# pyamg/pyamg

Hardware: AMD Instinct MI355X
Metric: vcycle_iterations_per_sec (higher is better)
Workload: dtype f64; 1 GPU; 3D 7-pt Poisson 256^3 (16.7M dof) SA V-cycle, symmetric Gauss-Seidel, fp64; key=c3, n=16777216, nnz=117047296, levels=5, cycle=V(1,1), graph=True, parallelism=1 GPU, gs_order=fast, full=False

## Files before the change

### pyamg_amd/csrc/pamg_common.h

```cpp
#pragma once
#include "pamg_host_threads.h"
#include <hip/hip_runtime.h>

#include <cstdint>
#include <cstdio>
#include <cstdlib>
#include <ctime>
#include <algorithm>
#include <atomic>
#include <cstring>
#include <thread>
#include <vector>

#include "../../include/pyamg_amd.h"

#define PAMG_STR2(x) #x
#define PAMG_STR(x) PAMG_STR2(x)
#define PAMG_HIP(expr)                                   \
    do {                                                 \
        hipError_t e__ = (expr);                         \
        if (e__ != hipSuccess) return (int)e__;          \
    } while (0)
#define PAMG_TRY(expr)                                   \
    do {                                                 \
// ... 149 lines not shown
    int use_rowg = 0;
    unsigned char *d_pid = nullptr;
    void *d_ptab = nullptr;
    int npat = 0, pat_lmax = 0;
    unsigned char *d_pmask = nullptr;
    int rm_nu = 0, rm_off[8] = {0, 0, 0, 0, 0, 0, 0, 0};
    unsigned long long rm_val[8] = {0, 0, 0, 0, 0, 0, 0, 0};
    long long rm_walked = 0;
    int rowmask_kz = 8;
    int rowmask_flags = 3;
    int use_rowpat = 1;
    int cap_from_val8 = 0;
    int stream_flags = 0;
    int lds_pad = 0;
    int gran_xcd = 0;
    int gran_cap = 0;
    int gs_mode = 0;
    int tile_G = 0;
    int tile_W = 0;
    int tile_cap = 0;
    int tile_D = 0, tile_Q = -1;
    int tile_part = 1;
    bool tile_default = false;
    int max_row_len = 0;
    int borrowed = 0;
    int gs_prof = 0;
    int gs_order = 0;
    int lane_L = 0, lane_G = 0;
    int lane_flags = 1;
    int line_scan = 1;
    int lane_merge = 0;
    int lanem_rpw = 0;
    int lanem_cluster = 0;
    int lanem_ahead10 = 40;
    int lane_wide = 0;
    int gs_cap = 0;
    int nblk = 0;
    int *d_part[2] = {nullptr, nullptr};
    int npart[2] = {0, 0};
    int64_t part_cols = -1;
    int64_t part_row0[2] = {-1, -1}, part_row1[2] = {-1, -1};
    int4 *d_blkmeta = nullptr;
    double *d_partial = nullptr;
    pamg::GsSchedule *gs[4] = {nullptr, nullptr, nullptr, nullptr};
    pamg_matrix_s *point_twin = nullptr;
    size_t point_twin_bytes = 0;
    bool point_twin_unfit = false;
    pamg::LineSchedule *ls[4] = {nullptr, nullptr, nullptr, nullptr};
    int sym_fused = 1;
    void *d_sym_hf[2] = {nullptr, nullptr}, *d_sym_hb = nullptr;
    unsigned *d_sym_sync = nullptr;
    int sym_cap = 0;
    const void *sym_cap_kernel = nullptr;
    int sym_form = 0, sym_grid = 0;
    long long sym_launches = 0, sym_zero_launches = 0;
    size_t bytes = 0;
};

struct pamg_schwarz_s;
struct pamg_solver_s;
struct pamg_csr_s;

namespace pamg {
int schwarz_sweep(pamg_schwarz_s *h, void *x, const void *b, int start, int stop, int step, hipStream_t s);
int schwarz_prepare(pamg_schwarz_s *h, int sweep);
int schwarz_error(pamg_schwarz_s *h, bool *error);
void schwarz_level_launches(pamg_schwarz_s *h);
int stream_launch(pamg_matrix_s *A, int epi, const void *x, const void *b, void *y, double c,
                  double omega, double *partial, hipStream_t s);
int stream_launch_part(pamg_matrix_s *A, int part, int epi, const void *x, const void *b, void *y, double c,
                       double omega, double *partial, hipStream_t s);
int matrix_split_ranges(pamg_matrix_s *A, int64_t n_owned_cols);
void matrix_drop_value_codes(pamg_matrix_s *A);
void matrix_drop_point_twin(pamg_matrix_s *A);
void matrix_drop_schedules(pamg_matrix_s *A);
int gs_sweep(pamg_matrix_s *A, int epi, void *x, const void *b, double omega, int row_start,
             int row_stop, int row_step, hipStream_t s);
int gs_sweep_symmetric(pamg_matrix_s *A, void *x, const void *b, bool x_zero, hipStream_t s, bool *ran);
int ensure_sym_parts(pamg_matrix_s *A);
int sym_reset(pamg_matrix_s *A);
int reduce_partials(const double *partial, int n, double *out, hipStream_t s);
int vec_sumsq(int dtype, int64_t n, const void *x, double *scratch, double *out, hipStream_t s);
int vec_axpy(int dtype, int64_t n, double a, const void *x, void *y, hipStream_t s);
int vec_scale(int dtype, int64_t n, double a, const void *x, void *y, hipStream_t s);
int vec_dot(int dtype, int64_t n, const void *x, const void *y, double *scratch, double *out, hipStream_t s);
int vec_mul(int dtype, int64_t n, const void *a, const void *b, void *y, hipStream_t s);
int kaczmarz_sweep(pamg_matrix_s *L, bool nr, void *v, const void *b, const void *Dinv, double omega, int start, int stop,
                   int step, void *xout, hipStream_t s);
int ensure_line_schedule(pamg_matrix_s *L, int start, int stop, int step);
void free_line_schedule(LineSchedule *g);
int vec_scatter(int dtype, int64_t n, const int *idx, const void *src, void *dst, hipStream_t s);
int vec_copy_indexed(int dtype, int64_t n, const int *idx, const void *src, void *dst, hipStream_t s);
int matrix_row_subset(pamg_matrix_s *A, const int32_t *rows, int nrows, pamg_matrix_s **out);
int jacobi_indexed(pamg_matrix_s *sub, void *x, const void *b, double omega, void *work, hipStream_t s);
int vec_maxratio(int dtype, int64_t n, const void *u, const void *x, double *scratch, double *out, hipStream_t s);
int vec_xpby(int dtype, int64_t n, double beta, const void *z, void *p, hipStream_t s);
int vec_axpy_ratio(int dtype, int64_t n, const double *num, const double *den, double sign, const void *x, void *y, hipStream_t s);
int vec_fill(int dtype, int64_t n, double v, void *y, hipStream_t s);
int dense_gemv(int dtype, int n, const void *M, const void *b, void *x, hipStream_t s);
int block_gs_sweep(pamg_matrix_s *A, void *x, const void *b, const void *Dinv, int row_start,
                   int row_stop, int row_step, hipStream_t s);
int block_jacobi_step(pamg_matrix_s *A, int kind, const void *Dinv, const void *xsrc, void *xdst,
                      const void *b, double omega, hipStream_t s);
int ensure_schedule(pamg_matrix_s *A, int row_start, int row_stop, int row_step, bool block_gs = false);
struct CsrArrays { int64_t m, n, nnz; const int *p, *j; const double *x; };
int csr_device_arrays(struct ::pamg_csr_s *A, CsrArrays *out);
constexpr int KR_PARTIALS = 3 * 2048;
int kr_reduce(int64_t n, const double *part, int k, double *o0, double *o1, double *o2, hipStream_t s);
// ... 5 lines not shown
               const void *AMs, void *r, const void *rstar, double *part, hipStream_t s);
int bicg_dir(int dtype, int64_t n, const double *rr_new, const double *rr_old, const double *alpha, const double *omega, const void *r,
             void *p, const void *AMp, void *bc, void *xc, hipStream_t s);
int cr_update(int dtype, int64_t n, const double *rAz, const double *ApAp, void *x, const void *p, void *r, const void *Ap, bool update_r,
              void *xc, hipStream_t s);
int cr_dir(int dtype, int64_t n, const double *rAz_new, const double *rAz_old, void *p, const void *z, void *Ap, const void *Az,
           double *part, hipStream_t s);
int sd_update(int dtype, int64_t n, const double *rz, const double *zAz, void *x, void *xc, void *r, const void *q, bool update_r,
              hipStream_t s);
int mr_update(int dtype, int64_t n, const double *pz, const double *pp, void *x, void *z, void *xc, bool update_z, double *part,
              hipStream_t s);
int kr_take(int dtype, int64_t n, void *xc, void *dst, double *part, hipStream_t s);
int solver_cycle_inline(pamg_solver_s *S, void *x, const void *b, int cycle, int cpl, hipStream_t s, bool allow_graph);
bool solver_needs_host_sync(const pamg_solver_s *S);
bool line_eligible(const pamg_matrix_s *A, const GsSchedule *g);
int build_line_part(pamg_matrix_s *A, GsSchedule *g);
void free_line_part(LineSched *t);
size_t line_part_bytes(const GsSchedule *g);
int line_launch(pamg_matrix_s *A, GsSchedule *g, int epi, void *x, const void *b, double omega, hipStream_t s);
int line_info(const GsSchedule *g, int64_t *info);
int line_sym_launch(pamg_matrix_s *A, GsSchedule *gf, GsSchedule *gb, void *x, const void *b, hipStream_t s);
int build_kz_lane_part(pamg_matrix_s *Lm, LineSchedule *g);
void free_kz_lane_part(KzLaneSched *t);
int kz_lane_launch(pamg_matrix_s *Lm, LineSchedule *g, bool nr, void *v, const void *b, const void *Dinv, double omega, void *xout, hipStream_t s);
int kz_lane_info(const LineSchedule *g, int64_t *info);
bool kz_lane_error(LineSchedule *g);
bool want_blanes(const pamg_matrix_s *A, const GsSchedule *g);
int block_point_sweep(pamg_matrix_s *A, GsSchedule *g, void *x, const void *b, int dirn, hipStream_t s);
int get_schedule(pamg_matrix_s *A, int row_start, int row_stop, int row_step, GsSchedule **out);
int ensure_parts(pamg_matrix_s *A, GsSchedule *g, bool block_gs = false);
int device_cus();
bool blane_eligible(const pamg_matrix_s *A, const GsSchedule *g);
int build_blane_part(pamg_matrix_s *A, GsSchedule *g);
void free_blane_part(BlaneSched *t);
size_t blane_part_bytes(const GsSchedule *g);
int blane_launch(pamg_matrix_s *A, GsSchedule *g, const void *Dinv, void *x, const void *b, hipStream_t s);
int blane_info(const GsSchedule *g, int64_t *info);
int blane_profile(const GsSchedule *g, long long *out, int64_t cap, int64_t *n);
int device_cus_lane();
bool lane_eligible(const pamg_matrix_s *A, const GsSchedule *g);
int build_lane_part(pamg_matrix_s *A, GsSchedule *g);
void free_lane_part(LaneSched *t);
size_t lane_part_bytes(const GsSchedule *g);
int lane_launch(pamg_matrix_s *A, GsSchedule *g, int epi, void *x, const void *b, double omega, hipStream_t s);
int lane_info(const GsSchedule *g, int64_t *info);
int lane_profile(const GsSchedule *g, long long *out, int64_t cap, int64_t *n);
int lanem_smax(const pamg_matrix_s *A, const GsSchedule *g);
int build_lanem_part(pamg_matrix_s *A, GsSchedule *g);
void free_lanem_part(struct LaneMSched *t);
size_t lanem_part_bytes(const GsSchedule *g);
int lanem_info(const GsSchedule *g, int64_t *info, double *growth);
int lanem_levels(const GsSchedule *g, int64_t *out, int64_t cap, int64_t *n);
int lanem_sym_launch(pamg_matrix_s *A, GsSchedule *gf, GsSchedule *gb, void *x, const void *b, bool x_zero, hipStream_t s);
int sym_fill_sentinels(void *p, int64_t n);
int sweep_error(pamg_matrix_s *A, bool *error);
inline size_t tsize(int dtype) { return dtype == PAMG_F64 ? 8 : 4; }

template <typename F>
inline void host_parallel(int64_t n, F fn, int64_t grain = 1 << 20)
{
    const unsigned hw = std::max(1u, std::min(32u, pamg::host_cpus()));
    const int nt = n < 2 * grain ? 1 : (int)std::min<int64_t>(hw, n / grain);
    if (nt <= 1) { fn((int64_t)0, n); return; }
    std::vector<std::thread> th;
    for (int t = 0; t < nt; ++t) {
        const int64_t lo = n * t / nt, hi = n * (t + 1) / nt;
        th.emplace_back([=] { fn(lo, hi); });
    }
    for (auto &x : th) x.join();
}

struct PhaseTimer {
    const char *name;
    int64_t items;
    timespec t0;
    static bool on() { static const int v = [] { const char *e = getenv("PAMG_TIMING"); return (e && *e && *e != '0') ? 1 : 0; }(); return v != 0; }
    explicit PhaseTimer(const char *n, int64_t k = 0) : name(n), items(k) { if (on()) clock_gettime(CLOCK_MONOTONIC, &t0); }
    ~PhaseTimer()
    {
        if (!on()) return;
        timespec t1;
        clock_gettime(CLOCK_MONOTONIC, &t1);
        fprintf(stderr, "[pamg timing] %-28s %8.3f s  (%lld)\n", name, (double)(t1.tv_sec - t0.tv_sec) + 1e-9 * (double)(t1.tv_nsec - t0.tv_nsec), (long long)items);
    }
};
}
```

### pyamg_amd/csrc/pamg_lane.hip

```cpp
#include "pamg_common.h"
#include "pamg_lane_plan.h"
#include "pamg_lanem_plan.h"

namespace pamg {

template <typename T> struct Sentinel;
template <> struct Sentinel<double> {
    using bits_t = unsigned long long;
    static constexpr bits_t value = 0x7FF8DEADBEEF5A5Aull;
    static __device__ __forceinline__ bits_t bits(double v) { return (bits_t)__double_as_longlong(v); }
};
template <> struct Sentinel<float> {
    using bits_t = unsigned int;
    static constexpr bits_t value = 0x7FC5BEEFu;
    static __device__ __forceinline__ bits_t bits(float v) { return __float_as_uint(v); }
};

template <typename T>
__global__ __launch_bounds__(BLK) void lane_fill_sentinel_kernel(T *xs, int64_t n)
{
    using B = typename Sentinel<T>::bits_t;
    B *p = reinterpret_cast<B *>(xs);
    for (int64_t i = (int64_t)blockIdx.x * BLK + threadIdx.x; i < n; i += (int64_t)gridDim.x * BLK) p[i] = Sentinel<T>::value;
}

struct alignas(16) LaneRec { int rid; int gate; int rd_lo; int rd_hi; };

struct LaneSched {
    int L = 0, K = 0, RPW = 0;
    int64_t ngroups = 0;
    int *d_cols = nullptr;
    LaneRec *d_rec = nullptr;
    void *d_vals = nullptr;
    long long *d_prof = nullptr;
    int64_t n_early = 0, n_old = 0, n_slots = 0;
    int64_t max_level_groups = 0;
    int last_grid = 0;
    int cap = 0;
    const void *cap_kernel = nullptr;
    size_t bytes = 0;
};

template <typename T>
struct LaneArgs {
    const int *cols;
    const T *vals;
    const LaneRec *rec;
    const T *x;
    T *y;
    T *xs;
    const T *b;
    unsigned *err;
    unsigned *ticket;
    long long *prof;
    int ngroups, nidle;
// ... 236 lines not shown
                lane_load<T, L, K>(a, g, P);
                if (lane == 0) tk4 = __hip_atomic_fetch_add(a.ticket, 1u, __ATOMIC_RELAXED, __HIP_MEMORY_SCOPE_AGENT);
            }
            lane_finish<T, EPI, L, K, MODE>(a, Q, D, g2, idle);
            if (g >= a.ngroups) break;
            g2 = (int)__builtin_amdgcn_readfirstlane(tk4);
        }
    }
}


struct alignas(32) LaneMRec { int rid_a; int rid_b; int gate; int unitK; int rda_lo; int rda_hi; int rdb_lo; int rdb_hi; };

struct LaneMSched {
    int64_t ngroups = 0, n_units = 0, nrows = 0;
    int rpw = 1;
    int nsuper = 0, nlevels = 0, s_max = 0, max_len = 0;
    int closed_by_length = 0, closed_by_growth = 0;
    double max_growth = 0.0;
    int64_t n_early = 0, n_old = 0, n_b = 0, max_super_groups = 0;
    int *d_cols = nullptr;
    double *d_vals = nullptr;
    LaneMRec *d_rec = nullptr;
    long long *d_prof = nullptr;
    int cluster = 0;
    int4 *d_crec = nullptr;
    unsigned short *d_sidx = nullptr;
    int *d_crid = nullptr;
    double *d_crd = nullptr;
    int64_t n_uunits = 0, n_uearly = 0, n_uold = 0, n_ub = 0, n_early_lines = 0;
    std::vector<int64_t> super_grp;
    int last_grid = 0;
    int cap = 0;
    const void *cap_kernel = nullptr;
    size_t bytes = 0;
};

struct LaneMArgs {
    const int *cols;
    const double *vals;
    const LaneMRec *rec;
    const double *xold;
    double *y;
    double *xs;
    const double *b;
    unsigned *err;
    unsigned *ticket;
    int ngroups, nidle, use_gate;
    long long *prof;
    const unsigned short *sidx;
    const int *crid;
    const double *crd;
    int crows;
};

__global__ __launch_bounds__(BLK) void lanem_prepare_kernel(const double *__restrict__ x, double *__restrict__ xold, double *__restrict__ xs, int64_t n)
{
    unsigned long long *p = reinterpret_cast<unsigned long long *>(xs);
    for (int64_t i = (int64_t)blockIdx.x * BLK + threadIdx.x; i < n; i += (int64_t)gridDim.x * BLK) {
        xold[i] = x[i];
        p[i] = Sentinel<double>::value;
    }
}

template <int NREG>
struct MCtx {
    int c[NREG];
    double v[NREG], xv[NREG];
    double bv, xo, rd;
    int rid;
    int gate, unit, K, g;
};

__device__ __forceinline__ void m_rec(const int4 *rp, int g, int gend, int4 &q0, int4 &q1)
{
    const size_t gg = (size_t)(g < gend ? g : gend - 1);
    q0 = rp[2 * gg];
    q1 = rp[2 * gg + 1];
}

template <int RPW, int NREG>
__device__ __forceinline__ void m_slots(const LaneMArgs &a, MCtx<NREG> &C, const int4 &q0, const int4 &q1, int g, int lane)
{
    C.g = g;
    const int rid_a = __builtin_amdgcn_readfirstlane(q0.x), rid_b = __builtin_amdgcn_readfirstlane(q0.y);
    C.gate = a.use_gate ? __builtin_amdgcn_readfirstlane(q0.z) : -1;
    const int uk = __builtin_amdgcn_readfirstlane(q0.w);
    C.unit = uk >> 4;
    C.K = uk & 15;
    const double rd_a = __hiloint2double(__builtin_amdgcn_readfirstlane(q1.y), __builtin_amdgcn_readfirstlane(q1.x));
    const double rd_b = __hiloint2double(__builtin_amdgcn_readfirstlane(q1.w), __builtin_amdgcn_readfirstlane(q1.z));
    const bool second = RPW == 2 && lane >= 32;
    C.rid = second ? rid_b : rid_a;
    C.rd = second ? rd_b : rd_a;
    const size_t e0 = (size_t)C.unit * 64 + (size_t)lane;
#pragma unroll
    for (int k = 0; k < NREG; ++k) {
        const size_t e = e0 + (size_t)64 * (size_t)(k < C.K ? k : C.K - 1);
        C.c[k] = a.cols[e];
        C.v[k] = a.vals[e];
    }
}

template <int NREG>
__device__ __forceinline__ void m_gather(const LaneMArgs &a, MCtx<NREG> &C, int idle, const bool xz = false, const bool coh = false)
{
#pragma unroll
    for (int k = 1; k < NREG; ++k)
        if (k >= C.K) C.c[k] = LANE_NONE;
    if (xz) {
#pragma unroll
        for (int k = 0; k < NREG; ++k)
            if (!(C.c[k] & (LANE_EARLY | LANEM_BSRC))) C.c[k] |= LANE_NONE;
    }
    const int row = C.rid < 0 ? 0 : (C.rid & LANE_MASK);
    C.bv = a.b[row];
    C.xo = coh ? __hip_atomic_load(a.xold + row, __ATOMIC_RELAXED, __HIP_MEMORY_SCOPE_AGENT) : a.xold[row];
#pragma unroll
    for (int k = 0; k < NREG; ++k) {
        const int col = C.c[k] & LANEM_MASK;
        const double *p = (C.c[k] & LANE_NONE) ? a.xold + idle : ((C.c[k] & LANE_EARLY) ? a.xs + col : ((C.c[k] & LANEM_BSRC) ? a.b + col : a.xold + col));
        C.xv[k] = __hip_atomic_load(p, __ATOMIC_RELAXED, __HIP_MEMORY_SCOPE_AGENT);
    }
}

template <int RPW, int NREG>
__device__ __forceinline__ double m_finish(const LaneMArgs &a, MCtx<NREG> &C, int idle, long long *t_ready = nullptr, unsigned *n_spins = nullptr, const bool xz = false)
{
    using T = double;
    const int lane = threadIdx.x & 63;
    unsigned pend = 0;
#pragma unroll
    for (int k = 0; k < NREG; ++k)
        if ((C.c[k] & LANE_EARLY) && !(C.c[k] & LANE_NONE) && Sentinel<T>::bits(C.xv[k]) == Sentinel<T>::value) pend |= 1u << k;
    unsigned spins = 0;
    if (C.gate >= 0 && __builtin_amdgcn_ballot_w64(pend != 0)) {
        const T *gp = a.xs + C.gate;
        while (true) {
            const T gv = __hip_atomic_load(gp, __ATOMIC_RELAXED, __HIP_MEMORY_SCOPE_AGENT);
            if (Sentinel<T>::bits(gv) != Sentinel<T>::value) break;
            __builtin_amdgcn_s_sleep(2);
            if ((++spins & 1023u) == 0 && (spins > (1u << 21) || __hip_atomic_load(a.err, __ATOMIC_RELAXED, __HIP_MEMORY_SCOPE_AGENT))) break;
        }
    }
    while (pend) {
        if (spins) __builtin_amdgcn_s_sleep(1);
        T t[NREG];
#pragma unroll
        for (int k = 0; k < NREG; ++k)
            t[k] = __hip_atomic_load(((pend >> k) & 1u) ? a.xs + (C.c[k] & LANEM_MASK) : a.xs + idle, __ATOMIC_RELAXED, __HIP_MEMORY_SCOPE_AGENT);
#pragma unroll
        for (int k = 0; k < NREG; ++k)
            if ((pend >> k) & 1u) {
                C.xv[k] = t[k];
                if (Sentinel<T>::bits(t[k]) != Sentinel<T>::value) pend &= ~(1u << k);
            }
        if ((++spins & 1023u) == 0) {
            if (spins > (1u << 21) || __hip_atomic_load(a.err, __ATOMIC_RELAXED, __HIP_MEMORY_SCOPE_AGENT)) {
                __hip_atomic_store(a.err, 1u, __ATOMIC_RELAXED, __HIP_MEMORY_SCOPE_AGENT);
                break;
            }
        }
    }
    if (t_ready) { *t_ready = wall_clock64(); *n_spins = spins; }
    T s = T(0);
#pragma unroll
    for (int k = 0; k < NREG; ++k) {
        const T pr = C.v[k] * C.xv[k];
        s = s + ((C.c[k] & LANE_NONE) ? T(0) : pr);
    }
    if (C.K > NREG) {
        for (int k = NREG; k < C.K; ++k) {
            const size_t e = (size_t)(C.unit + k) * 64 + (size_t)lane;
            int c = a.cols[e];
            if (xz && !(c & (LANE_EARLY | LANEM_BSRC))) c |= LANE_NONE;
            const T v = a.vals[e];
            const int col = c & LANEM_MASK;
            const bool early = (c & LANE_EARLY) && !(c & LANE_NONE);
            const T *p = (c & LANE_NONE) ? a.xold + idle : ((c & LANE_EARLY) ? a.xs + col : ((c & LANEM_BSRC) ? a.b + col : a.xold + col));
            T x = __hip_atomic_load(p, __ATOMIC_RELAXED, __HIP_MEMORY_SCOPE_AGENT);
            unsigned sp2 = 0;
            while (__builtin_amdgcn_ballot_w64(early && Sentinel<T>::bits(x) == Sentinel<T>::value)) {
                __builtin_amdgcn_s_sleep(1);
                const T t = __hip_atomic_load(p, __ATOMIC_RELAXED, __HIP_MEMORY_SCOPE_AGENT);
                if (early && Sentinel<T>::bits(x) == Sentinel<T>::value) x = t;
                if ((++sp2 & 1023u) == 0 && (sp2 > (1u << 21) || __hip_atomic_load(a.err, __ATOMIC_RELAXED, __HIP_MEMORY_SCOPE_AGENT))) {
                    __hip_atomic_store(a.err, 1u, __ATOMIC_RELAXED, __HIP_MEMORY_SCOPE_AGENT);
                    break;
                }
            }
            const T pr = v * x;
            s = s + ((c & LANE_NONE) ? T(0) : pr);
        }
    }
    s = seg_allreduce<64 / RPW, T>(s);
    const bool upd = C.rid >= 0 && !(C.rid & LANE_NODIAG);
    T val = (C.bv - s) * C.rd;
    if (!upd) val = C.xo;
    return val;
}

template <int RPW, int MODE, int NREG, int PH = 0>
__device__ __forceinline__ void m_publish(const LaneMArgs &a, const MCtx<NREG> &C, double val)
{
    if (((threadIdx.x & 63) & (64 / RPW - 1)) == 0 && C.rid >= 0) {
        const int row = C.rid & LANE_MASK;
        if constexpr (MODE == 1) __hip_atomic_store(a.xs + row, val, __ATOMIC_RELAXED, __HIP_MEMORY_SCOPE_WORKGROUP);
        else __hip_atomic_store(a.xs + row, val, __ATOMIC_RELAXED, __HIP_MEMORY_SCOPE_AGENT);
        if constexpr (PH != 1) {
            if (!(C.rid & LANE_NODIAG)) a.y[row] = val;
        }
    }
}

constexpr int LANEC_K = 8;

__device__ __forceinline__ int4 c_rec(const int4 *rp, int g, int gend) { return rp[(size_t)(g < gend ? g : gend - 1)]; }

template <int PH>
__device__ __forceinline__ void c_group(const LaneMArgs &a, double *lds, const int4 &q, int g, int lane, int idle, const bool xz, const bool coh)
{
    using T = double;
    const int gate = a.use_gate ? __builtin_amdgcn_readfirstlane(q.x) : -1;
    const int uunit = __builtin_amdgcn_readfirstlane(q.y), sunit = __builtin_amdgcn_readfirstlane(q.z), kk = __builtin_amdgcn_readfirstlane(q.w);
    const int KU = kk & 15, KS = (kk >> 8) & 15;
    int c[LANEC_K];
    unsigned si[LANEC_K];
    T sv[LANEC_K], xv[LANEC_K];
    const size_t u0 = (size_t)uunit * 64 + (size_t)lane, s0 = (size_t)sunit * 64 + (size_t)lane;
#pragma unroll
    for (int k = 0; k < LANEC_K; ++k) {
        c[k] = LANE_NONE;
        if (k < KU) c[k] = a.cols[u0 + (size_t)64 * k];
    }
#pragma unroll
    for (int k = 0; k < LANEC_K; ++k) {
        si[k] = LANEC_PAD | LANEC_UNUSED; sv[k] = T(0);
        if (k < KS) { si[k] = a.sidx[s0 + (size_t)64 * k]; sv[k] = a.vals[s0 + (size_t)64 * k]; }
    }
    if (xz) {
#pragma unroll
        for (int k = 0; k < LANEC_K; ++k)
            if (!(c[k] & (LANE_EARLY | LANEM_BSRC))) c[k] |= LANE_NONE;
    }
#pragma unroll
    for (int k = 0; k < LANEC_K; ++k) {
        xv[k] = T(0);
        if (k < KU) {
            const int col = c[k] & LANEM_MASK;
            const T *p = (c[k] & LANE_NONE) ? a.xold + idle : ((c[k] & LANE_EARLY) ? a.xs + col : ((c[k] & LANEM_BSRC) ? a.b + col : a.xold + col));
            xv[k] = __hip_atomic_load(p, __ATOMIC_RELAXED, __HIP_MEMORY_SCOPE_AGENT);
        }
    }
    const bool unused = (si[0] & LANEC_UNUSED) != 0;
    const int tag = (int)((si[0] >> LANEC_ROWSHIFT) & 7u);
    const size_t ri = (size_t)g * (size_t)a.crows + (size_t)(tag < a.crows ? tag : 0);
    const int rid = unused ? -1 : a.crid[ri];
    const T rd = a.crd[ri];
    const int row = rid < 0 ? 0 : (rid & LANE_MASK);
    const T bv = a.b[row];
    const T xo = coh ? __hip_atomic_load(a.xold + row, __ATOMIC_RELAXED, __HIP_MEMORY_SCOPE_AGENT) : a.xold[row];
    unsigned pend = 0;
#pragma unroll
    for (int k = 0; k < LANEC_K; ++k)
        if ((c[k] & LANE_EARLY) && !(c[k] & LANE_NONE) && Sentinel<T>::bits(xv[k]) == Sentinel<T>::value) pend |= 1u << k;
    unsigned spins = 0;
    if (gate >= 0 && __builtin_amdgcn_ballot_w64(pend != 0)) {
        const T *gp = a.xs + gate;
        while (true) {
            const T gv = __hip_atomic_load(gp, __ATOMIC_RELAXED, __HIP_MEMORY_SCOPE_AGENT);
            if (Sentinel<T>::bits(gv) != Sentinel<T>::value) break;
            __builtin_amdgcn_s_sleep(2);
            if ((++spins & 1023u) == 0 && (spins > (1u << 21) || __hip_atomic_load(a.err, __ATOMIC_RELAXED, __HIP_MEMORY_SCOPE_AGENT))) break;
        }
    }
    while (pend) {
        if (spins) __builtin_amdgcn_s_sleep(1);
        T t[LANEC_K];
#pragma unroll
        for (int k = 0; k < LANEC_K; ++k) {
            t[k] = T(0);
            if (k < KU) t[k] = __hip_atomic_load(((pend >> k) & 1u) ? a.xs + (c[k] & LANEM_MASK) : a.xs + idle, __ATOMIC_RELAXED, __HIP_MEMORY_SCOPE_AGENT);
        }
#pragma unroll
        for (int k = 0; k < LANEC_K; ++k)
            if ((pend >> k) & 1u) {
                xv[k] = t[k];
                if (Sentinel<T>::bits(t[k]) != Sentinel<T>::value) pend &= ~(1u << k);
            }
        if ((++spins & 1023u) == 0) {
            if (spins > (1u << 21) || __hip_atomic_load(a.err, __ATOMIC_RELAXED, __HIP_MEMORY_SCOPE_AGENT)) {
                __hip_atomic_store(a.err, 1u, __ATOMIC_RELAXED, __HIP_MEMORY_SCOPE_AGENT);
                break;
            }
        }
    }
#pragma unroll
    for (int k = 0; k < LANEC_K; ++k)
        if (k < KU) lds[k * 64 + lane] = (c[k] & LANE_NONE) ? T(0) : xv[k];
    __builtin_amdgcn_fence(__ATOMIC_RELEASE, "wavefront");
    __builtin_amdgcn_wave_barrier();
    __builtin_amdgcn_fence(__ATOMIC_ACQUIRE, "wavefront");
    T s = T(0);
#pragma unroll
    for (int k = 0; k < LANEC_K; ++k) {
        const T pr = sv[k] * lds[si[k] & LANEC_IDX];
        s = s + ((si[k] & LANEC_PAD) ? T(0) : pr);
    }
    const unsigned key = si[0] & ((7u << LANEC_ROWSHIFT) | LANEC_UNUSED);
    const unsigned left = (unsigned)__shfl_up((int)key, 1);
    const unsigned long long heads = __builtin_amdgcn_ballot_w64(lane == 0 || left != key);
    const int seglo = 63 - __builtin_clzll(heads & (~0ull >> (63 - lane)));
#pragma unroll
    for (int d = 1; d < 64; d *= 2) {
        const T o = __shfl_up(s, d);
        s = s + ((lane - d >= seglo) ? o : T(0));
    }
    const bool tail = ((((heads >> 1) | (1ull << 63)) >> lane) & 1ull) != 0;
    __builtin_amdgcn_fence(__ATOMIC_RELEASE, "wavefront");
    __builtin_amdgcn_wave_barrier();
    const bool upd = rid >= 0 && !(rid & LANE_NODIAG);
    T val = (bv - s) * rd;
    if (!upd) val = xo;
    if (tail && rid >= 0) {
        __hip_atomic_store(a.xs + row, val, __ATOMIC_RELAXED, __HIP_MEMORY_SCOPE_AGENT);
        if constexpr (PH != 1) {
            if (upd) a.y[row] = val;
        }
    }
}

template <int MODE, int RPW, int NREG>
__global__ __launch_bounds__(BLK) void gs_lanem_kernel(const LaneMArgs a)
{
    const int lane = threadIdx.x & 63;
    const int wib = threadIdx.x >> 6;
    const int idle = (int)((((unsigned)blockIdx.x * LANE_WPB + (unsigned)wib) * 16u) % (unsigned)a.nidle);
    const int4 *rp = reinterpret_cast<const int4 *>(a.rec);
    const int gend = a.ngroups;
    __shared__ double c_lds[RPW == 0 ? LANE_WPB * LANEC_UMAX : 1];
    if constexpr (RPW == 0) {
        static_assert(RPW != 0 || MODE != 1, "the cluster layout has no ticket form");
        const int W = (int)gridDim.x * LANE_WPB;
        int g = __builtin_amdgcn_readfirstlane((int)blockIdx.x * LANE_WPB + wib);
        if (g >= gend) return;
        int4 q = c_rec(rp, g, gend);
        for (; g < gend; g += W) {
            const int4 nq = c_rec(rp, g + W, gend);
            c_group<0>(a, c_lds + wib * LANEC_UMAX, q, g, lane, idle, false, false);
            q = nq;
        }
    } else {
    MCtx<NREG> X;
    if constexpr (MODE != 1) {
        const int W = (int)gridDim.x * LANE_WPB;
        int g = __builtin_amdgcn_readfirstlane((int)blockIdx.x * LANE_WPB + wib);
        if (g >= gend) return;
        int4 q0, q1;
        m_rec(rp, g, gend, q0, q1);
        for (; g < gend; g += W) {
            int4 n0, n1;
            m_rec(rp, g + W, gend, n0, n1);
            if (a.prof) {
                const long long t0 = wall_clock64();
                m_slots<RPW, NREG>(a, X, q0, q1, g, lane);
                asm volatile("s_waitcnt vmcnt(0)" ::: "memory");
                const long long t1 = wall_clock64();
                m_gather<NREG>(a, X, idle);
                long long t2 = 0;
                unsigned sp = 0;
                const double val = m_finish<RPW, NREG>(a, X, idle, &t2, &sp);
                m_publish<RPW, MODE, NREG>(a, X, val);
                if (lane == 0) {
                    long long *o = a.prof + (size_t)g * 4;
                    o[0] = t0 | ((long long)(sp > 4095u ? 4095u : sp) << 52);
                    o[1] = t1; o[2] = t2; o[3] = wall_clock64();
                }
            } else {
                m_slots<RPW, NREG>(a, X, q0, q1, g, lane);
                m_gather<NREG>(a, X, idle);
                const double val = m_finish<RPW, NREG>(a, X, idle);
                m_publish<RPW, MODE, NREG>(a, X, val);
            }
            q0 = n0; q1 = n1;
        }
    } else {
        __shared__ int sh_home;
        if (threadIdx.x == 0) {
            const unsigned me = (__builtin_amdgcn_s_getreg((3 << 11) | 20) & 0xF) + 1u;
            unsigned home = 0u;
            __hip_atomic_compare_exchange_strong(a.ticket + 1, &home, me, __ATOMIC_RELAXED, __ATOMIC_RELAXED, __HIP_MEMORY_SCOPE_AGENT);
            sh_home = (home == 0u || home == me) ? 1 : 0;
        }
        __syncthreads();
        if (!sh_home) return;
        unsigned tk = 0;
        if (lane == 0) tk = __hip_atomic_fetch_add(a.ticket, 1u, __ATOMIC_RELAXED, __HIP_MEMORY_SCOPE_AGENT);
        int g = (int)__builtin_amdgcn_readfirstlane(tk);
        if (g >= gend) return;
        if (lane == 0) tk = __hip_atomic_fetch_add(a.ticket, 1u, __ATOMIC_RELAXED, __HIP_MEMORY_SCOPE_AGENT);
        int g2 = (int)__builtin_amdgcn_readfirstlane(tk);
        int4 q0, q1;
        m_rec(rp, g, gend, q0, q1);
        while (true) {
            int4 n0, n1;
            m_rec(rp, g2, gend, n0, n1);
            unsigned tk3 = 0;
            if (g2 < gend && lane == 0) tk3 = __hip_atomic_fetch_add(a.ticket, 1u, __ATOMIC_RELAXED, __HIP_MEMORY_SCOPE_AGENT);
            m_slots<RPW, NREG>(a, X, q0, q1, g, lane);
            m_gather<NREG>(a, X, idle);
            const double val = m_finish<RPW, NREG>(a, X, idle);
            m_publish<RPW, MODE, NREG>(a, X, val);
            if (g2 >= gend) break;
            g = g2; q0 = n0; q1 = n1;
            g2 = (int)__builtin_amdgcn_readfirstlane(tk3);
        }
    }
    }
}

struct LaneMSymArgs {
    LaneMArgs ph[2];
    double *hf[2];
    unsigned *sync;
    int wq[2], wr[2], wblk[2];
    int xzero;
};

template <int MODE>
__device__ __forceinline__ void m_wipe(double *w, int g, int G, int q, int r, int blk, int lane)
{
    if (g & (blk - 1)) return;
    const int g1 = g + blk < G ? g + blk : G;
    const int lo = g * q + (g < r ? g : r), hi = g1 * q + (g1 < r ? g1 : r);
    unsigned long long *p = reinterpret_cast<unsigned long long *>(w);
    for (int i = lo + lane; i < hi; i += 64) {
        if constexpr (MODE == 1) __hip_atomic_store(p + i, Sentinel<double>::value, __ATOMIC_RELAXED, __HIP_MEMORY_SCOPE_WORKGROUP);
        else __hip_atomic_store(p + i, Sentinel<double>::value, __ATOMIC_RELAXED, __HIP_MEMORY_SCOPE_AGENT);
    }
}

template <int MODE, int RPW, int NREG, int PH>
__device__ __forceinline__ unsigned m_phase(const LaneMArgs &a, double *wipe, int wq, int wr, int wblk, unsigned *ticket, const bool xz, int lane, int wib, int idle, double *c_lds)
{
    const int4 *rp = reinterpret_cast<const int4 *>(a.rec);
    const int gend = a.ngroups;
    unsigned done = 0;
    if constexpr (RPW == 0) {
        static_assert(RPW != 0 || MODE != 1, "the cluster layout has no ticket form");
        const int W = (int)gridDim.x * LANE_WPB;
        int g = __builtin_amdgcn_readfirstlane((int)blockIdx.x * LANE_WPB + wib);
        if (g >= gend) return 0;
        int4 q = c_rec(rp, g, gend);
        for (; g < gend; g += W) {
            const int4 nq = c_rec(rp, g + W, gend);
            c_group<PH>(a, c_lds + wib * LANEC_UMAX, q, g, lane, idle, xz, PH == 2);
            m_wipe<MODE>(wipe, g, gend, wq, wr, wblk, lane);
            ++done;
            q = nq;
        }
    } else {
    MCtx<NREG> X;
    if constexpr (MODE != 1) {
        const int W = (int)gridDim.x * LANE_WPB;
        int g = __builtin_amdgcn_readfirstlane((int)blockIdx.x * LANE_WPB + wib);
        if (g >= gend) return 0;
        int4 q0, q1;
        m_rec(rp, g, gend, q0, q1);
        for (; g < gend; g += W) {
            int4 n0, n1;
            m_rec(rp, g + W, gend, n0, n1);
            m_slots<RPW, NREG>(a, X, q0, q1, g, lane);
            m_gather<NREG>(a, X, idle, xz, PH == 2);
            const double val = m_finish<RPW, NREG>(a, X, idle, nullptr, nullptr, xz);
            m_publish<RPW, MODE, NREG, PH>(a, X, val);
            m_wipe<MODE>(wipe, g, gend, wq, wr, wblk, lane);
            ++done;
            q0 = n0; q1 = n1;
        }
    } else {
        unsigned tk = 0;
        if (lane == 0) tk = __hip_atomic_fetch_add(ticket, 1u, __ATOMIC_RELAXED, __HIP_MEMORY_SCOPE_AGENT);
        int g = (int)__builtin_amdgcn_readfirstlane(tk);
        if (g >= gend) return 0;
        if (lane == 0) tk = __hip_atomic_fetch_add(ticket, 1u, __ATOMIC_RELAXED, __HIP_MEMORY_SCOPE_AGENT);
        int g2 = (int)__builtin_amdgcn_readfirstlane(tk);
        int4 q0, q1;
        m_rec(rp, g, gend, q0, q1);
        while (true) {
            int4 n0, n1;
            m_rec(rp, g2, gend, n0, n1);
            unsigned tk3 = 0;
            if (g2 < gend && lane == 0) tk3 = __hip_atomic_fetch_add(ticket, 1u, __ATOMIC_RELAXED, __HIP_MEMORY_SCOPE_AGENT);
            m_slots<RPW, NREG>(a, X, q0, q1, g, lane);
            m_gather<NREG>(a, X, idle, xz, PH == 2);
            const double val = m_finish<RPW, NREG>(a, X, idle, nullptr, nullptr, xz);
            m_publish<RPW, MODE, NREG, PH>(a, X, val);
            m_wipe<MODE>(wipe, g, gend, wq, wr, wblk, lane);
            ++done;
            if (g2 >= gend) break;
            g = g2; q0 = n0; q1 = n1;
            g2 = (int)__builtin_amdgcn_readfirstlane(tk3);
        }
    }
    }
    return done;
}

__device__ __forceinline__ void sym_phase_barrier(unsigned *counter, unsigned *err, unsigned *sh_done, unsigned done, unsigned total)
{
    asm volatile("s_waitcnt vmcnt(0)" ::: "memory");
    if ((threadIdx.x & 63) == 0 && done) atomicAdd(sh_done, done);
    __syncthreads();
    if (threadIdx.x == 0) {
        const unsigned mine = *sh_done;
        if (mine) __hip_atomic_fetch_add(counter, mine, __ATOMIC_RELAXED, __HIP_MEMORY_SCOPE_AGENT);
        unsigned spins = 0;
        while (__hip_atomic_load(counter, __ATOMIC_RELAXED, __HIP_MEMORY_SCOPE_AGENT) < total) {
            __builtin_amdgcn_s_sleep(2);
            if ((++spins & 1023u) == 0 && (spins > (1u << 21) || __hip_atomic_load(err, __ATOMIC_RELAXED, __HIP_MEMORY_SCOPE_AGENT))) {
                __hip_atomic_store(err, 1u, __ATOMIC_RELAXED, __HIP_MEMORY_SCOPE_AGENT);
                break;
            }
        }
    }
    __syncthreads();
}

__device__ __forceinline__ void sym_leave(unsigned *sync, unsigned parity)
{
    __syncthreads();
    if (threadIdx.x == 0) {
        const unsigned left = __hip_atomic_fetch_add(sync + 1, 1u, __ATOMIC_RELAXED, __HIP_MEMORY_SCOPE_AGENT);
        if (left == gridDim.x - 1) {
            for (int k = 0; k < 5; ++k) __hip_atomic_store(sync + k, 0u, __ATOMIC_RELAXED, __HIP_MEMORY_SCOPE_AGENT);
            __hip_atomic_store(sync + 5, parity ^ 1u, __ATOMIC_RELAXED, __HIP_MEMORY_SCOPE_AGENT);
        }
    }
}

template <int MODE, int RPW, int NREG>
__global__ __launch_bounds__(BLK) void gs_lanem_sym_kernel(const LaneMSymArgs a)
{
    __shared__ unsigned sh_done;
    __shared__ int sh_home;
    __shared__ double c_lds[RPW == 0 ? LANE_WPB * LANEC_UMAX : 1];
    const int lane = threadIdx.x & 63;
    const int wib = threadIdx.x >> 6;
    const int idle = (int)((((unsigned)blockIdx.x * LANE_WPB + (unsigned)wib) * 16u) % (unsigned)a.ph[0].nidle);
    const unsigned parity = __builtin_amdgcn_readfirstlane(__hip_atomic_load(a.sync + 5, __ATOMIC_RELAXED, __HIP_MEMORY_SCOPE_AGENT)) & 1u;
    if (threadIdx.x == 0) {
        sh_done = 0u;
        sh_home = 1;
        if constexpr (MODE == 1) {
            const unsigned me = (__builtin_amdgcn_s_getreg((3 << 11) | 20) & 0xF) + 1u;
            unsigned home = 0u;
            __hip_atomic_compare_exchange_strong(a.sync + 4, &home, me, __ATOMIC_RELAXED, __ATOMIC_RELAXED, __HIP_MEMORY_SCOPE_AGENT);
            sh_home = (home == 0u || home == me) ? 1 : 0;
        }
    }
    __syncthreads();
    if (sh_home) {
        double *hf = a.hf[parity], *hf_next = a.hf[parity ^ 1u];
        LaneMArgs p1 = a.ph[0], p2 = a.ph[1];
        p1.xs = hf; p1.y = nullptr;
        p2.xold = hf;
        const unsigned done = m_phase<MODE, RPW, NREG, 1>(p1, p2.xs, a.wq[0], a.wr[0], a.wblk[0], a.sync + 2, a.xzero != 0, lane, wib, idle, c_lds);
        sym_phase_barrier(a.sync, p1.err, &sh_done, done, (unsigned)p1.ngroups);
        (void)m_phase<MODE, RPW, NREG, 2>(p2, hf_next, a.wq[1], a.wr[1], a.wblk[1], a.sync + 3, false, lane, wib, idle, c_lds);
    }
    sym_leave(a.sync, parity);
}

namespace {

template <typename U>
int lane_upload(U **dst, const void *src, size_t bytes, size_t *total)
{
    *dst = nullptr;
    const size_t alloc = std::max<size_t>(bytes, 256) + 256;
    PAMG_HIP(hipMalloc((void **)dst, alloc));
    if (bytes && src) PAMG_HIP(hipMemcpy(*dst, src, bytes, hipMemcpyHostToDevice));
    if (total) *total += alloc;
    return PAMG_OK;
}

template <typename T, int EPI, int L, int MODE>
const void *lane_kernel_k(int K)
{
    switch (K) {
        case 1: return (const void *)gs_lane_kernel<T, EPI, L, 1, MODE>;
        case 2: return (const void *)gs_lane_kernel<T, EPI, L, 2, MODE>;
        case 3: return (const void *)gs_lane_kernel<T, EPI, L, 3, MODE>;
        case 4: return (const void *)gs_lane_kernel<T, EPI, L, 4, MODE>;
    }
    return nullptr;
}

template <typename T, int EPI, int MODE>
const void *lane_kernel_l(int L, int K)
{
    switch (L) {
        case 4: return lane_kernel_k<T, EPI, 4, MODE>(K);
        case 8: return lane_kernel_k<T, EPI, 8, MODE>(K);
        case 16: return lane_kernel_k<T, EPI, 16, MODE>(K);
        case 32: return lane_kernel_k<T, EPI, 32, MODE>(K);
        case 64: return lane_kernel_k<T, EPI, 64, MODE>(K);
    }
    return nullptr;
}

template <typename T>
const void *lane_kernel(int epi, int L, int K, int mode)
{
    if (epi == EPI_SOR) return mode == 1 ? lane_kernel_l<T, EPI_SOR, 1>(L, K) : lane_kernel_l<T, EPI_SOR, 0>(L, K);
    return mode == 1 ? lane_kernel_l<T, EPI_GS, 1>(L, K) : lane_kernel_l<T, EPI_GS, 0>(L, K);
}

}

void free_lane_part(LaneSched *t)
{
// ... 110 lines not shown
        if (!st) st = lane_upload(&t->d_vals, nullptr, (size_t)P.n_slots * ts, &t->bytes);
        if (!st) {
            const unsigned grid = (unsigned)((P.ngroups + 3) / 4);
            (void)hipGetLastError();
            if (ts == 8)
                hipLaunchKernelGGL((lane_fill_kernel<double>), dim3(grid), dim3(256), 0, 0, (int)A->nrows, A->d_Ap, A->d_Aj, (const double *)A->d_Ax, g->row_start, g->row_step,
                                   (long long)g->nrows, P.L, P.K, (long long)P.ngroups, d_rid, d_gate, t->d_cols, (double *)t->d_vals, t->d_rec);
            else
                hipLaunchKernelGGL((lane_fill_kernel<float>), dim3(grid), dim3(256), 0, 0, (int)A->nrows, A->d_Ap, A->d_Aj, (const float *)A->d_Ax, g->row_start, g->row_step,
                                   (long long)g->nrows, P.L, P.K, (long long)P.ngroups, d_rid, d_gate, t->d_cols, (float *)t->d_vals, t->d_rec);
            st = (int)hipGetLastError();
            if (!st) st = (int)hipDeviceSynchronize();
        }
        hipFree(d_rid); hipFree(d_gate);
    }
    if (st) { free_lane_part(t); return st; }
    g->lane = t;
    g->bytes += t->bytes;
    return PAMG_OK;
}

size_t lane_part_bytes(const GsSchedule *g) { return (g && g->lane) ? g->lane->bytes : 0; }

void free_lanem_part(LaneMSched *t)
{
    if (!t) return;
    hipFree(t->d_cols); hipFree(t->d_vals); hipFree(t->d_rec); hipFree(t->d_prof);
    hipFree(t->d_crec); hipFree(t->d_sidx); hipFree(t->d_crid); hipFree(t->d_crd);
    delete t;
}

size_t lanem_part_bytes(const GsSchedule *g) { return (g && g->lanem) ? g->lanem->bytes : 0; }

int lanem_cluster_rows(const pamg_matrix_s *A)
{
    if (A->lanem_cluster >= 4) return A->lanem_cluster;
    if (A->lanem_cluster == 1) return 0;
    static const int env = [] { const char *e = getenv("PAMG_LANEM_CLUSTER"); return e ? atoi(e) : 0; }();
    if (A->nrows <= 131072 || env == 1) return 0;
    return env == 4 ? 4 : 8;
}

int lanem_smax(const pamg_matrix_s *A, const GsSchedule *g)
{
    if (A->dtype != PAMG_F64 || A->R != 1 || g->nlevels < 8) return 1;
    if (A->lane_merge == 1) return 1;
    if (A->lane_merge >= 2) return A->lane_merge;
    const char *e = getenv("PAMG_LANE_MERGE");
    if (e && atoi(e) >= 1) return atoi(e);
    if (A->nnz < 12 * std::max<int64_t>(1, A->nrows)) return 1;
    return A->nrows > 131072 ? (lanem_cluster_rows(A) ? 4 : 3) : 8;
}

int build_lanem_part(pamg_matrix_s *A, GsSchedule *g)
{
    if (g->lanem) return PAMG_OK;
    const int s_max = lanem_smax(A, g);
    if (s_max < 2) return PAMG_E_ARG;
    PhaseTimer pt_("build_lanem_part", A->nnz);
    PlanVec<double> hAx;
    hAx.resize((size_t)A->nnz + 1);
    if (A->nnz) PAMG_HIP(hipMemcpy(hAx.data(), A->d_Ax, (size_t)A->nnz * sizeof(double), hipMemcpyDeviceToHost));
    LaneMPlan P;
    const int rpw = A->lanem_rpw ? A->lanem_rpw : (A->nrows > 131072 ? 2 : 1);
    const int cluster = lanem_cluster_rows(A);
    if (build_lanem_plan((int)A->nrows, A->h_Ap.data(), A->h_Aj.data(), hAx.data(), g->row_start, g->row_step, (int)g->nrows, g->nlevels, g->h_vis, g->h_lvl,
                         s_max, 1e3, P, LANEM_KMAX * 64, rpw, cluster))
        return PAMG_E_ARG;
    hAx = PlanVec<double>();
    if (P.nsuper * 10 > P.nlevels * 9) return PAMG_E_ARG;
    LaneMSched *t = new (std::nothrow) LaneMSched();
    if (!t) return PAMG_E_ALLOC;
    t->ngroups = P.ngroups; t->n_units = P.n_units; t->nrows = P.nrows; t->rpw = P.rpw; t->nsuper = P.nsuper; t->nlevels = P.nlevels; t->s_max = s_max; t->max_len = P.max_len;
    t->closed_by_length = P.closed_by_length; t->closed_by_growth = P.closed_by_growth; t->max_growth = P.max_growth;
    t->n_early = P.n_early; t->n_old = P.n_old; t->n_b = P.n_b; t->max_super_groups = P.max_super_groups;
    t->super_grp = P.super_grp;
    t->cluster = P.cluster; t->n_uunits = P.n_uunits; t->n_uearly = P.n_uearly; t->n_uold = P.n_uold; t->n_ub = P.n_ub; t->n_early_lines = P.n_early_lines;
    if (P.cluster) {
        std::vector<int4> crec((size_t)P.ngroups);
        lane_parallel(P.ngroups, [&](int64_t g0, int64_t g1) {
            for (int64_t q = g0; q < g1; ++q)
                crec[(size_t)q] = make_int4(P.gate[(size_t)q], P.c_uunit[(size_t)q], P.c_sunit[(size_t)q],
                                            (int)P.c_KU[(size_t)q] | ((int)P.c_KS[(size_t)q] << 8) | ((int)P.c_rows[(size_t)q] << 16));
        });
        int st = lane_upload(&t->d_crec, crec.data(), crec.size() * sizeof(int4), &t->bytes);
        if (!st) st = lane_upload(&t->d_cols, P.ucodes.data(), P.ucodes.size() * sizeof(int), &t->bytes);
        if (!st) st = lane_upload(&t->d_vals, P.svals.data(), P.svals.size() * sizeof(double), &t->bytes);
        if (!st) st = lane_upload(&t->d_sidx, P.sidx.data(), P.sidx.size() * sizeof(unsigned short), &t->bytes);
        if (!st) st = lane_upload(&t->d_crid, P.rid.data(), P.rid.size() * sizeof(int), &t->bytes);
        if (!st) st = lane_upload(&t->d_crd, P.rdiag.data(), P.rdiag.size() * sizeof(double), &t->bytes);
        if (!st && !g->d_xold) {
            const size_t xb = ((size_t)A->nrows + 8) * sizeof(double);
            st = (int)hipMalloc(&g->d_xold, xb);
            if (!st) t->bytes += xb;
        }
        if (st) { free_lanem_part(t); return st; }
        if (getenv("PAMG_TIMING")) fprintf(stderr, "[pamg timing]     lanem plan: cluster layout, %d rows per wave: %zu bytes uploaded\n", P.cluster, t->bytes);
        g->lanem = t;
        g->bytes += t->bytes;
        return PAMG_OK;
    }
    std::vector<LaneMRec> rec((size_t)P.ngroups);
    lane_parallel(P.ngroups, [&](int64_t g0, int64_t g1) {
        for (int64_t q = g0; q < g1; ++q) {
            LaneMRec &R = rec[(size_t)q];
            const size_t q0 = (size_t)q * (size_t)P.rpw;
            const double zero = 0.0;
            R.rid_a = P.rid[q0]; R.rid_b = P.rpw == 2 ? P.rid[q0 + 1] : -1;
            R.gate = P.gate[(size_t)q];
            R.unitK = P.unit[(size_t)q] * 16 + (int)P.K[(size_t)q];
            std::memcpy(&R.rda_lo, &P.rdiag[q0], 8);
            std::memcpy(&R.rdb_lo, P.rpw == 2 ? &P.rdiag[q0 + 1] : &zero, 8);
        }
    });
    int st = lane_upload(&t->d_rec, rec.data(), rec.size() * sizeof(LaneMRec), &t->bytes);
    if (!st) st = lane_upload(&t->d_cols, P.cols.data(), P.cols.size() * sizeof(int), &t->bytes);
    if (!st) st = lane_upload(&t->d_vals, P.vals.data(), P.vals.size() * sizeof(double), &t->bytes);
    if (!st && !g->d_xold) {
        const size_t xb = ((size_t)A->nrows + 8) * sizeof(double);
        st = (int)hipMalloc(&g->d_xold, xb);
        if (!st) t->bytes += xb;
    }
    if (st) { free_lanem_part(t); return st; }
    if (getenv("PAMG_TIMING")) fprintf(stderr, "[pamg timing]     lanem plan: %d row(s) per wave: %zu bytes uploaded\n", P.rpw, t->bytes);
    g->lanem = t;
    g->bytes += t->bytes;
    return PAMG_OK;
}

static void lanem_layout_args(const LaneMSched *t, LaneMArgs &a)
{
    a.cols = t->d_cols; a.vals = t->d_vals;
    a.rec = t->cluster ? reinterpret_cast<const LaneMRec *>(t->d_crec) : t->d_rec;
    a.sidx = t->d_sidx; a.crid = t->d_crid; a.crd = t->d_crd; a.crows = t->cluster;
}

int lanem_launch(pamg_matrix_s *A, GsSchedule *g, void *x, const void *b, hipStream_t s)
{
    LaneMSched *t = g->lanem;
    if (!t || !g->d_xold) return PAMG_E_STATE;
    const int64_t n = A->nrows;
    LaneMArgs a;
    lanem_layout_args(t, a);
    a.use_gate = (A->lane_flags & 1) ? 1 : 0;
    a.xold = (const double *)g->d_xold; a.y = (double *)x; a.xs = (double *)g->d_xs; a.b = (const double *)b;
    a.err = g->d_sync + 1; a.ticket = g->d_sync + 20;
    a.ngroups = (int)t->ngroups;
    a.nidle = (int)std::max<int64_t>(1, std::min<int64_t>(n, 1 << 20));
    if (A->gs_prof && !t->d_prof && !t->cluster) {
        PAMG_HIP(hipMalloc((void **)&t->d_prof, (size_t)t->ngroups * 4 * sizeof(long long)));
        PAMG_HIP(hipMemset(t->d_prof, 0, (size_t)t->ngroups * 4 * sizeof(long long)));
    }
    a.prof = (A->gs_prof && !t->cluster) ? t->d_prof : nullptr;
    const int fgrid = (int)std::min<int64_t>(4096, (n + BLK - 1) / BLK);
    hipLaunchKernelGGL(lanem_prepare_kernel, dim3(fgrid), dim3(BLK), 0, s, (const double *)x, (double *)g->d_xold, (double *)g->d_xs, n);
    PAMG_HIP(hipGetLastError());
    const bool xcd = !t->cluster && (A->gran_xcd == 1 || (A->gran_xcd == 0 && lane_one_xcd(A, g) && A->nrows <= 8192));
    static const int nreg_env = [] { const char *e = getenv("PAMG_LANEM_NREG"); return e ? atoi(e) : 0; }();
    const bool all_regs = t->rpw == 1 && (nreg_env ? nreg_env == 8 : A->nrows <= 131072);
    const void *k = t->cluster  ? (const void *)gs_lanem_kernel<0, 0, 8>
                  : t->rpw == 2 ? (xcd ? (const void *)gs_lanem_kernel<1, 2, 4> : (const void *)gs_lanem_kernel<0, 2, 4>)
                  : all_regs    ? (xcd ? (const void *)gs_lanem_kernel<1, 1, 8> : (const void *)gs_lanem_kernel<0, 1, 8>)
                                : (xcd ? (const void *)gs_lanem_kernel<1, 1, 2> : (const void *)gs_lanem_kernel<0, 1, 2>);
    static thread_local int cus = 0;
    if (!cus) cus = device_cus_lane();
    if (!(t->cap > 0 && t->cap_kernel == k)) {
        int nb = 0;
        if (hipOccupancyMaxActiveBlocksPerMultiprocessor(&nb, k, BLK, 0) != hipSuccess) nb = 2;
        t->cap = std::max(1, std::min(nb - 1, 8));
        t->cap_kernel = k;
    }
    const int cap = t->cap;
    const int per_level = (int)((t->ngroups + t->nsuper - 1) / std::max(1, t->nsuper));
    const int64_t want_waves = std::max<int64_t>(128, ((int64_t)A->lanem_ahead10 * per_level + 9) / 10);
    const int cwpb = LANE_WPB;
    int G = (int)std::min<int64_t>((want_waves + cwpb - 1) / cwpb, (int64_t)std::min(cap, (t->rpw == 2 || t->cluster) ? 2 : 3) * cus);
    if (A->lane_G > 0) G = std::min(A->lane_G, cap * cus);
    G = (int)std::max<int64_t>(1, std::min<int64_t>(G, (t->ngroups + cwpb - 1) / cwpb));
    void *args[] = {(void *)&a};
    if (xcd) {
        PAMG_HIP(hipMemsetAsync(g->d_sync + 20, 0, 2 * sizeof(unsigned), s));
        const int Gx = std::max(1, std::min(G, (cus / 8) * cap));
        t->last_grid = 8 * Gx;
        PAMG_HIP(hipLaunchKernel(k, dim3(8 * Gx), dim3(BLK), args, 0, s));
        return PAMG_OK;
    }
    t->last_grid = G;
    PAMG_HIP(hipLaunchKernel(k, dim3(G), dim3(BLK), args, 0, s));
    return PAMG_OK;
}

int sym_fill_sentinels(void *p, int64_t n)
{
    if (n <= 0) return PAMG_OK;
    const int fgrid = (int)std::min<int64_t>(4096, (n + BLK - 1) / BLK);
    hipLaunchKernelGGL((lane_fill_sentinel_kernel<double>), dim3(fgrid), dim3(BLK), 0, 0, (double *)p, n);
    PAMG_HIP(hipGetLastError());
    PAMG_HIP(hipDeviceSynchronize());
    return PAMG_OK;
}

int lanem_sym_launch(pamg_matrix_s *A, GsSchedule *gf, GsSchedule *gb, void *x, const void *b, bool x_zero, hipStream_t s)
{
    LaneMSched *tf = gf->lanem, *tb = gb->lanem;
    if (!tf || !tb || !A->d_sym_hf[0] || !A->d_sym_hf[1] || !A->d_sym_hb || !A->d_sym_sync) return PAMG_E_STATE;
    const int64_t n = A->nrows;
    auto one_xcd = [&](const GsSchedule *g) { return !g->lanem->cluster && (A->gran_xcd == 1 || (A->gran_xcd == 0 && lane_one_xcd(A, g) && A->nrows <= 8192)); };
    const bool xcd = one_xcd(gf);
    if (xcd != one_xcd(gb) || tf->rpw != tb->rpw || tf->cluster != tb->cluster || tf->ngroups < 1 || tb->ngroups < 1) return PAMG_E_UNSUPPORTED;
    LaneMSymArgs a;
    GsSchedule *gs2[2] = {gf, gb};
    for (int p = 0; p < 2; ++p) {
        LaneMSched *t = gs2[p]->lanem;
        LaneMArgs &q = a.ph[p];
        lanem_layout_args(t, q);
        q.use_gate = (A->lane_flags & 1) ? 1 : 0;
        q.b = (const double *)b;
        q.err = gf->d_sync + 1; q.ticket = nullptr;
        q.ngroups = (int)t->ngroups;
        q.nidle = (int)std::max<int64_t>(1, std::min<int64_t>(n, 1 << 20));
        q.prof = nullptr;
        a.wq[p] = (int)(n / t->ngroups); a.wr[p] = (int)(n % t->ngroups);
        a.wblk[p] = 1;
        while ((int64_t)a.wblk[p] * n < 64 * t->ngroups && a.wblk[p] < (1 << 20)) a.wblk[p] *= 2;
    }
    a.ph[0].xold = (const double *)x; a.ph[0].y = nullptr;     a.ph[0].xs = nullptr;
    a.ph[1].xold = nullptr;           a.ph[1].y = (double *)x; a.ph[1].xs = (double *)A->d_sym_hb;
    a.hf[0] = (double *)A->d_sym_hf[0]; a.hf[1] = (double *)A->d_sym_hf[1];
    a.sync = A->d_sym_sync;
    a.xzero = x_zero ? 1 : 0;
    static const int nreg_env = [] { const char *e = getenv("PAMG_LANEM_NREG"); return e ? atoi(e) : 0; }();
    const bool all_regs = tf->rpw == 1 && (nreg_env ? nreg_env == 8 : A->nrows <= 131072);
    const void *k = tf->cluster  ? (const void *)gs_lanem_sym_kernel<0, 0, 8>
                  : tf->rpw == 2 ? (xcd ? (const void *)gs_lanem_sym_kernel<1, 2, 4> : (const void *)gs_lanem_sym_kernel<0, 2, 4>)
                  : all_regs     ? (xcd ? (const void *)gs_lanem_sym_kernel<1, 1, 8> : (const void *)gs_lanem_sym_kernel<0, 1, 8>)
                                 : (xcd ? (const void *)gs_lanem_sym_kernel<1, 1, 2> : (const void *)gs_lanem_sym_kernel<0, 1, 2>);
    static thread_local int cus = 0;
    if (!cus) cus = device_cus_lane();
    if (!(A->sym_cap > 0 && A->sym_cap_kernel == k)) {
        int nb = 0;
        if (hipOccupancyMaxActiveBlocksPerMultiprocessor(&nb, k, BLK, 0) != hipSuccess) nb = 2;
        A->sym_cap = std::max(1, std::min(nb - 1, 8));
        A->sym_cap_kernel = k;
    }
    const int cap = A->sym_cap;
    int G = 1;
    for (int p = 0; p < 2; ++p) {
        const LaneMSched *t = gs2[p]->lanem;
        const int per_level = (int)((t->ngroups + t->nsuper - 1) / std::max(1, t->nsuper));
        const int64_t want_waves = std::max<int64_t>(128, ((int64_t)A->lanem_ahead10 * per_level + 9) / 10);
        int Gp = (int)std::min<int64_t>((want_waves + LANE_WPB - 1) / LANE_WPB, (int64_t)std::min(cap, (t->rpw == 2 || t->cluster) ? 2 : 3) * cus);
        if (A->lane_G > 0) Gp = std::min(A->lane_G, cap * cus);
        Gp = (int)std::max<int64_t>(1, std::min<int64_t>(Gp, (t->ngroups + LANE_WPB - 1) / LANE_WPB));
        G = std::max(G, Gp);
    }
    if (xcd) G = 8 * std::max(1, std::min(G, (cus / 8) * cap));
    void *args[] = {(void *)&a};
    PAMG_HIP(hipLaunchKernel(k, dim3(G), dim3(BLK), args, 0, s));
    A->sym_form = xcd ? 3 : 1; A->sym_grid = G;
    A->sym_launches++;
    if (x_zero) A->sym_zero_launches++;
    return PAMG_OK;
}

int lanem_info(const GsSchedule *g, int64_t *info, double *growth)
{
    for (int i = 0; i < 20; ++i) info[i] = 0;
    if (growth) *growth = 0.0;
    if (!g || !g->lanem) return PAMG_OK;
    const LaneMSched *t = g->lanem;
    info[0] = t->nsuper; info[1] = t->nlevels; info[2] = t->nrows; info[3] = t->n_units; info[4] = t->n_early; info[5] = t->n_old; info[6] = t->n_b;
    info[7] = t->max_len; info[8] = t->s_max; info[9] = t->closed_by_length; info[10] = t->closed_by_growth; info[11] = t->last_grid;
    info[12] = t->cluster; info[13] = t->ngroups; info[14] = t->n_units * 64; info[15] = t->n_uunits;
    info[16] = t->cluster ? t->n_uearly : t->n_early; info[17] = t->cluster ? t->n_uold : t->n_old; info[18] = t->cluster ? t->n_ub : t->n_b; info[19] = t->n_early_lines;
    if (growth) *growth = t->max_growth;
    return PAMG_OK;
}


static int lane_grid_cap(LaneSched *t, const void *k)
{
    if (t->cap > 0 && t->cap_kernel == k) return t->cap;
    int nb = 0;
    if (hipOccupancyMaxActiveBlocksPerMultiprocessor(&nb, k, BLK, 0) != hipSuccess) nb = 2;
    nb = std::max(1, std::min(nb - 1, 8));
    t->cap = nb; t->cap_kernel = k;
    return nb;
}

int device_cus_lane()
{
    int dev = 0;
    hipDeviceProp_t p;
    if (hipGetDevice(&dev) != hipSuccess || hipGetDeviceProperties(&p, dev) != hipSuccess) return 64;
    return p.multiProcessorCount;
}

template <typename T>
static int lane_launch_t(pamg_matrix_s *A, GsSchedule *g, int epi, void *x, const void *b, double omega, hipStream_t s)
{
    LaneSched *t = g->lane;
    const size_t ts = tsize(A->dtype);
    const int64_t n = A->nrows;
    LaneArgs<T> a;
    a.cols = t->d_cols; a.vals = (const T *)t->d_vals; a.rec = t->d_rec;
    a.use_gate = (A->lane_flags & 1) ? 1 : 0;
    a.x = (const T *)x; a.y = (T *)x; a.xs = (T *)g->d_xs; a.b = (const T *)b;
    a.err = g->d_sync + 1; a.ticket = g->d_sync + 20;
    a.ngroups = (int)t->ngroups;
    a.nidle = (int)std::max<int64_t>(1, std::min<int64_t>(n, 1 << 20));
    a.omega = (T)omega;
    if (!g->symmetric) {
        if (!g->d_xold) return PAMG_E_STATE;
        PAMG_HIP(hipMemcpyAsync(g->d_xold, x, (size_t)n * ts, hipMemcpyDeviceToDevice, s));
        a.x = (const T *)g->d_xold;
    }
    if (A->gs_prof && !t->d_prof) {
        PAMG_HIP(hipMalloc((void **)&t->d_prof, (size_t)t->ngroups * 4 * sizeof(long long)));
        PAMG_HIP(hipMemset(t->d_prof, 0, (size_t)t->ngroups * 4 * sizeof(long long)));
    }
    a.prof = A->gs_prof ? t->d_prof : nullptr;
    const int fgrid = (int)std::min<int64_t>(4096, (n + BLK - 1) / BLK);
    hipLaunchKernelGGL((lane_fill_sentinel_kernel<T>), dim3(fgrid), dim3(BLK), 0, s, (T *)g->d_xs, n);
// ... 68 lines not shown
```

### pyamg_amd/csrc/pamg_matrix.hip

```cpp
#include "pamg_host_threads.h"
#include <algorithm>
#include <atomic>
#include <mutex>
#include <climits>
#include <new>
#include <thread>

#include "pamg_kernels.h"
#include "pamg_tile_kernels.h"
#include "pamg_tile_plan.h"
#include "pamg_stream_plan.h"

using namespace pamg;

namespace {

constexpr int PAD = 8;

std::mutex g_sched_mu;

template <typename U>
int upload(U **dptr, const U *h, size_t n, size_t *bytes)
{
    const size_t sz = (n + PAD) * sizeof(U);
// ... 745 lines not shown
    a.Aj16 = nullptr;
    a.wbase = nullptr;
    a.wb = make_int4(0, 0, 0, 0);
    a.blkmap = nullptr;
    a.Ax8 = nullptr;
    a.vdict = nullptr;
    a.nvd = 0;
    a.pid = nullptr;
    a.ptab = nullptr;
    a.npat = a.lmax = 0;
    return a;
}

double *g_scratch = nullptr;
int g_scratch_dev = -1;

}

namespace pamg {

void matrix_drop_value_codes(pamg_matrix_s *A) { if (A) drop_val8(A); }

void matrix_drop_point_twin(pamg_matrix_s *A)
{
    if (!A) return;
    pamg_matrix_s *T = nullptr;
    {
        std::lock_guard<std::mutex> lk(g_sched_mu);
        T = A->point_twin;
        if (T) A->bytes -= std::min(A->bytes, A->point_twin_bytes);
        A->point_twin = nullptr;
        A->point_twin_bytes = 0;
        A->point_twin_unfit = false;
    }
    if (T) pamg_matrix_destroy(T);
}

void matrix_drop_schedules(pamg_matrix_s *A)
{
    if (!A) return;
    for (int k = 0; k < 4; ++k) {
        GsSchedule *g = nullptr;
        LineSchedule *l = nullptr;
        {
            std::lock_guard<std::mutex> lk(g_sched_mu);
            g = A->gs[k]; l = A->ls[k];
            if (g) A->bytes -= std::min(A->bytes, g->bytes);
            if (l) A->bytes -= std::min(A->bytes, l->bytes);
            A->gs[k] = nullptr; A->ls[k] = nullptr;
        }
        free_schedule(g);
        if (l) free_line_schedule(l);
    }
    matrix_drop_point_twin(A);
}

int matrix_split_ranges(pamg_matrix_s *A, int64_t n_owned_cols)
{
    if (!A || n_owned_cols < 0) return PAMG_E_ARG;
    for (int k = 0; k < 2; ++k) { if (A->d_part[k]) { hipFree(A->d_part[k]); A->d_part[k] = nullptr; } A->npart[k] = 0; A->part_row0[k] = A->part_row1[k] = -1; }
    A->part_cols = -1;
    if (A->nblk == 0 || A->h_Ap.empty()) { A->part_cols = n_owned_cols; return PAMG_OK; }
    std::vector<int4> blk;
    blk.reserve((size_t)A->nblk);
    plan_rows(A->h_Ap.data(), 0, (int)A->nrows, A->cap, A->max_rows, blk);
    if ((int)blk.size() != A->nblk) return PAMG_E_STATE;
    std::vector<unsigned char> bnd(blk.size(), 0);
    const int *Aj = A->h_Aj.data();
    const int lim = (int)std::min<int64_t>(n_owned_cols, INT_MAX);
    parallel_rows((int)blk.size(), [&](int lo, int hi) {
        for (int b = lo; b < hi; ++b) {
            unsigned char any = 0;
            for (int p = blk[b].z; p < blk[b].w && !any; ++p) any = Aj[p] >= lim;
            bnd[(size_t)b] = any;
        }
    });
    std::vector<int> part[2];
    for (int b = 0; b < (int)blk.size(); ++b) part[bnd[(size_t)b] ? 1 : 0].push_back(b);
    for (int k = 0; k < 2; ++k) {
        A->npart[k] = (int)part[k].size();
        PAMG_TRY(upload(&A->d_part[k], part[k].data(), part[k].size(), &A->bytes));
        A->part_row0[k] = A->part_row1[k] = -1;
        if (!part[k].empty() && part[k].back() - part[k].front() + 1 == (int)part[k].size()) {
            A->part_row0[k] = blk[(size_t)part[k].front()].x;
            A->part_row1[k] = blk[(size_t)part[k].back()].y;
        }
    }
    A->part_cols = n_owned_cols;
    return PAMG_OK;
}

int stream_launch(pamg_matrix_s *A, int epi, const void *x, const void *b, void *y, double c,
                  double omega, double *partial, hipStream_t s)
{
    return stream_launch_part(A, 0, epi, x, b, y, c, omega, partial, s);
}

int stream_launch_part(pamg_matrix_s *A, int part, int epi, const void *x, const void *b, void *y, double c,
                       double omega, double *partial, hipStream_t s)
{
    if (part < 0 || part > 2) return PAMG_E_ARG;
    if (part && A->part_cols < 0) return PAMG_E_STATE;
    if (part) {
        const int n = A->npart[part - 1];
        if (n == 0) return PAMG_OK;
        const bool idx16 = A->use_idx16 && A->d_Aj16 && A->npl == 2;
// ... 396 lines not shown
    if (ensure_parts(A, gf) != PAMG_OK || ensure_parts(A, gb) != PAMG_OK) return 0;
    if (gf->nrows != A->nrows || gb->nrows != A->nrows) return 0;
    *pf = gf; *pb = gb;
    const bool lf = want_lines(A, gf), lb = want_lines(A, gb);
    if (lf != lb) return 0;
    if (lf) return (gf->line && gb->line && gf->symmetric && gb->symmetric) ? 2 : 0;
    if (want_lanes(A, gf) && want_lanes(A, gb) && gf->lanem && gb->lanem) return 1;
    return 0;
}

int ensure_sym_parts(pamg_matrix_s *A)
{
    GsSchedule *gf = nullptr, *gb = nullptr;
    if (!A || A->d_sym_hf[0] || !sym_form_of(A, &gf, &gb)) return PAMG_OK;
    const size_t vb = ((size_t)A->nrows + 8) * sizeof(double);
    void *hf0 = nullptr, *hf1 = nullptr, *hb = nullptr;
    unsigned *sy = nullptr;
    int st = (int)hipMalloc(&hf0, vb);
    if (!st) st = (int)hipMalloc(&hf1, vb);
    if (!st) st = (int)hipMalloc(&hb, vb);
    if (!st) st = (int)hipMalloc((void **)&sy, 16 * sizeof(unsigned));
    if (!st) st = (int)hipMemset(sy, 0, 16 * sizeof(unsigned));
    if (!st) st = sym_fill_sentinels(hf0, A->nrows + 8);
    if (!st) st = sym_fill_sentinels(hf1, A->nrows + 8);
    if (!st) st = sym_fill_sentinels(hb, A->nrows + 8);
    if (st) { hipFree(hf0); hipFree(hf1); hipFree(hb); hipFree(sy); return st; }
    A->d_sym_hf[0] = hf0; A->d_sym_hf[1] = hf1; A->d_sym_hb = hb; A->d_sym_sync = sy;
    { std::lock_guard<std::mutex> lk(g_sched_mu); A->bytes += 3 * vb + 16 * sizeof(unsigned); }
    return PAMG_OK;
}

int sym_reset(pamg_matrix_s *A)
{
    if (!A || !A->d_sym_hf[0]) return PAMG_OK;
    PAMG_HIP(hipDeviceSynchronize());
    PAMG_HIP(hipMemset(A->d_sym_sync, 0, 16 * sizeof(unsigned)));
    PAMG_TRY(sym_fill_sentinels(A->d_sym_hf[0], A->nrows + 8));
    return sym_fill_sentinels(A->d_sym_hf[1], A->nrows + 8);
}

int gs_sweep_symmetric(pamg_matrix_s *A, void *x, const void *b, bool x_zero, hipStream_t s, bool *ran)
{
    *ran = false;
    GsSchedule *gf = nullptr, *gb = nullptr;
    const int form = sym_form_of(A, &gf, &gb);
    if (!form) return PAMG_OK;
    if (!A->d_sym_hf[0]) {
        hipStreamCaptureStatus cs = hipStreamCaptureStatusNone;
        PAMG_HIP(hipStreamIsCapturing(s, &cs));
        if (cs != hipStreamCaptureStatusNone) return PAMG_OK;
        PAMG_TRY(ensure_sym_parts(A));
        if (!A->d_sym_hf[0]) return PAMG_OK;
    }
    const int st = form == 2 ? line_sym_launch(A, gf, gb, x, b, s) : lanem_sym_launch(A, gf, gb, x, b, x_zero, s);
    if (st == PAMG_E_UNSUPPORTED) return PAMG_OK;
    if (st == PAMG_OK) *ran = true;
    return st;
}

int ensure_schedule(pamg_matrix_s *A, int row_start, int row_stop, int row_step, bool block_gs)
{
    GsSchedule *g = nullptr;
    PAMG_TRY(get_schedule(A, row_start, row_stop, row_step, &g));
    return ensure_parts(A, g, block_gs);
}

int reduce_partials(const double *partial, int n, double *out, hipStream_t s)
{
    if (n > 8192) {
        double *mid = const_cast<double *>(partial) + n;
        hipLaunchKernelGGL(reduce_mid_kernel, dim3(256), dim3(BLK), 0, s, partial, n, mid);
        hipLaunchKernelGGL(reduce_final_kernel, dim3(1), dim3(BLK), 0, s, (const double *)mid, 256, out);
    } else {
        hipLaunchKernelGGL(reduce_final_kernel, dim3(1), dim3(BLK), 0, s, partial, n, out);
    }
    return (int)hipGetLastError();
}

int vec_sumsq(int dtype, int64_t n, const void *x, double *scratch, double *out, hipStream_t s)
{
    const int grid = (int)std::min<int64_t>(1024, std::max<int64_t>(1, (n + BLK - 1) / BLK));
    if (dtype == PAMG_F64)
        hipLaunchKernelGGL((vec_sumsq_kernel<double>), dim3(grid), dim3(BLK), 0, s, (const double *)x, n, scratch);
    else
        hipLaunchKernelGGL((vec_sumsq_kernel<float>), dim3(grid), dim3(BLK), 0, s, (const float *)x, n, scratch);
    PAMG_HIP(hipGetLastError());
    return reduce_partials(scratch, grid, out, s);
}

int vec_dot(int dtype, int64_t n, const void *x, const void *y, double *scratch, double *out, hipStream_t s)
{
    const int grid = (int)std::min<int64_t>(1024, std::max<int64_t>(1, (n + BLK - 1) / BLK));
    if (dtype == PAMG_F64)
        hipLaunchKernelGGL((vec_dot_kernel<double>), dim3(grid), dim3(BLK), 0, s, (const double *)x, (const double *)y, n, scratch);
    else
        hipLaunchKernelGGL((vec_dot_kernel<float>), dim3(grid), dim3(BLK), 0, s, (const float *)x, (const float *)y, n, scratch);
    PAMG_HIP(hipGetLastError());
    hipLaunchKernelGGL(reduce_final_kernel, dim3(1), dim3(BLK), 0, s, (const double *)scratch, grid, out);
    return (int)hipGetLastError();
}

static int vgrid(int64_t n) { return (int)std::min<int64_t>(1 << 21, std::max<int64_t>(1, (n + BLK - 1) / BLK)); }

int vec_mul(int dtype, int64_t n, const void *a, const void *b, void *y, hipStream_t s)
{
    if (n <= 0) return PAMG_OK;
    const int grid = vgrid(n);
// ... 366 lines not shown
            A->h_bAp.assign(Ap, Ap + n_brow + 1);
            A->h_bAj.assign(Aj, Aj + nblk);
            A->nblocks_b = nblk;
            st = upload(&A->d_bAp, A->h_bAp.data(), A->h_bAp.size(), &A->bytes);
            if (!st) st = upload(&A->d_bAj, A->h_bAj.data(), A->h_bAj.size(), &A->bytes);
            if (!st) st = upload_raw(&A->d_bAx, Ax, (size_t)A->nnz, ts, &A->bytes);
            std::vector<int> bjf(A->h_bAj), bdiag((size_t)n_brow, -1);
            for (int i = 0; i < n_brow; ++i)
                for (int p = Ap[i]; p < Ap[i + 1]; ++p)
                    if (Aj[p] == i) { bjf[p] = i | 0x40000000; bdiag[i] = p; }
            if (!st) st = upload(&A->d_bAjf, bjf.data(), bjf.size(), &A->bytes);
            if (!st) st = upload(&A->d_bdiag, bdiag.data(), bdiag.size(), &A->bytes);
        }
    }
    if (!st) {
        std::atomic<int> mx(0);
        host_parallel(A->nrows, [&](int64_t lo, int64_t hi) {
            int m = 0;
            for (int64_t i = lo; i < hi; ++i) m = std::max(m, A->h_Ap[i + 1] - A->h_Ap[i]);
            int cur = mx.load();
            while (m > cur && !mx.compare_exchange_weak(cur, m)) {}
        });
        A->max_row_len = mx.load();
    }
    A->cap = 1536; A->npl = 2; A->max_rows = 1024;
    if (A->d_Ax8 && R == 1 && C == 1) {
        const int64_t avg = (A->nnz + A->nrows - 1) / std::max<int64_t>(1, A->nrows);
        const int64_t rows = std::min<int64_t>(512, std::max<int64_t>(64, ((A->nrows / 2048 + 63) / 64) * 64));
        A->max_rows = (int)rows;
        A->cap = (int)std::min<int64_t>(12288, std::max<int64_t>(512, ((rows * avg + 255) / 256) * 256));
        A->cap_from_val8 = 1;
        A->use_rowg = 1;
    }
    if (!st) st = replan(A);
    if (!st && A->d_Ax8 && !A->d_Aj16) {
        drop_val8(A);
        A->cap = 1536; A->max_rows = 1024; A->cap_from_val8 = 0; A->use_rowg = 0;
        st = replan(A);
    }
    if (st) { pamg_matrix_destroy(A); return st; }
    *out = A;
    return PAMG_OK;
}

int pamg_matrix_destroy(pamg_matrix_t A)
{
    if (!A) return PAMG_OK;
    hipFree(A->d_Ap); hipFree(A->d_Aj); hipFree(A->d_Ax); hipFree(A->d_diag); hipFree(A->d_rowid);
    hipFree(A->d_bAp); hipFree(A->d_bAj); hipFree(A->d_bAjf); hipFree(A->d_bdiag); hipFree(A->d_bAx); hipFree(A->d_blkmeta); hipFree(A->d_partial); hipFree(A->d_bmeta); hipFree(A->d_Aj16); hipFree(A->d_wbase); hipFree(A->d_Ax8); hipFree(A->d_vdict); hipFree(A->d_pid); hipFree(A->d_ptab);
    hipFree(A->d_part[0]); hipFree(A->d_part[1]);
    for (int k = 0; k < 4; ++k) free_schedule(A->gs[k]);
    for (int k = 0; k < 4; ++k) pamg::free_line_schedule(A->ls[k]);
    hipFree(A->d_sym_hf[0]); hipFree(A->d_sym_hf[1]); hipFree(A->d_sym_hb); hipFree(A->d_sym_sync);
    if (A->point_twin) pamg_matrix_destroy(A->point_twin);
    delete A;
    return PAMG_OK;
}

int pamg_matrix_point_twin(pamg_matrix_t A, int *state)
{
    if (!A || !state) return PAMG_E_ARG;
    *state = A->point_twin_unfit ? 2 : A->point_twin ? 1 : 0;
    return PAMG_OK;
}

int pamg_matrix_info(pamg_matrix_t A, int64_t info[8])
{
    if (!A || !info) return PAMG_E_ARG;
    info[0] = A->nrows; info[1] = A->ncols; info[2] = A->nnz; info[3] = A->nblk;
    info[4] = A->cap; info[5] = (int64_t)A->bytes;
    info[6] = info[7] = 0;
    const int n = A->R > 1 ? A->n_brow : (int)A->nrows;
    for (int k = 0; k < 4; ++k) {
        GsSchedule *g = A->gs[k];
        if (!g) continue;
        if (g->row_start == 0 && g->row_stop == n && g->row_step == 1) info[6] = g->nlevels;
        if (g->row_start == n - 1 && g->row_stop == -1 && g->row_step == -1) info[7] = g->nlevels;
    }
    return PAMG_OK;
}

int pamg_matrix_value_codes(pamg_matrix_t A, int *n_values)
{
    if (!A || !n_values) return PAMG_E_ARG;
    *n_values = (A->d_Ax8 && A->use_val8 && A->use_idx16 && A->d_Aj16 && A->npl == 2) ? A->nvdict : 0;
    return PAMG_OK;
}

int pamg_matrix_row_patterns(pamg_matrix_t A, int *n_patterns)
{
    if (!A || !n_patterns) return PAMG_E_ARG;
    *n_patterns = (A->d_pid && A->use_rowpat && A->d_Ax8 && A->use_val8 && A->use_idx16 && A->d_Aj16 && A->npl == 2) ? A->npat : 0;
    return PAMG_OK;
}

int pamg_matrix_row_masks(pamg_matrix_t A, long long info[8])
{
    if (!A || !info) return PAMG_E_ARG;
    for (int k = 0; k < 8; ++k) info[k] = 0;
    int npat = 0;
    pamg_matrix_row_patterns(A, &npat);
    if (!npat || !A->d_pmask || (A->use_rowpat != 1 && A->use_rowpat != 4)) return PAMG_OK;
    info[0] = A->rm_nu; info[1] = A->rm_walked; info[5] = A->rowmask_kz; info[6] = A->rowmask_flags;
    info[7] = (A->nrows + BLK - 1) / BLK;
    RowMaskLattice g;
    int grid3 = 0;
    if (A->use_rowpat == 1 && rowmask_lattice_plan(A->rm_nu, A->rm_off, A->nrows, A->rowmask_kz, (A->rowmask_flags & 2) != 0, false, g, grid3)) {
        info[2] = 1; info[3] = g.L; info[4] = g.P; info[7] = grid3;
    }
    return PAMG_OK;
}

int pamg_matrix_tune(pamg_matrix_t A, int key, int value)
{
    if (!A) return PAMG_E_ARG;
    if (key == 21) { A->use_val8 = value != 0; return PAMG_OK; }
    if (key == 22) { A->use_rowg = value != 0; return PAMG_OK; }
    if (key == 23) { if (value < 0 || value > 4 || value == 2) return PAMG_E_ARG; A->use_rowpat = value; return PAMG_OK; }
    if (A->borrowed > 0) return PAMG_E_STATE;
    switch (key) {
        case 0: if (value < 64 || value > 12288) return PAMG_E_ARG; A->cap = value & ~3; A->cap_from_val8 = 0; break;
        case 1: if (value != 2) return PAMG_E_ARG; A->npl = 2; return PAMG_OK;
        case 2: if (value < 1) return PAMG_E_ARG; A->max_rows = value; break;
        case 3: if (value < 0 || value > 256) return PAMG_E_ARG; A->flow_cap = value; return PAMG_OK;
        case 5: if (value < 0 || value > 5) return PAMG_E_ARG; A->gs_mode = value; return PAMG_OK;
        case 6: if (value < 0) return PAMG_E_ARG; A->gran_cap = value; return PAMG_OK;
        case 7: if (value < 0 || value > 2) return PAMG_E_ARG; A->gran_xcd = value; matrix_drop_point_twin(A); return PAMG_OK;
        case 8: if (value < 0 || value > 63) return PAMG_E_ARG; A->stream_flags = value; return PAMG_OK;
        case 11: A->gs_prof = value != 0; return PAMG_OK;
        case 12: if (value < 0) return PAMG_E_ARG; A->tile_G = value; break;
        case 13: if (value != 0 && (value < 64 || value > 8192 || (value & (value - 1)))) return PAMG_E_ARG; A->tile_W = value; break;
        case 14: if (value < 0 || value > TILE_MAX_ENTRIES) return PAMG_E_ARG; A->tile_cap = value; break;
        case 15: A->tile_default = value != 0; return PAMG_OK;
        case 16: if (value < 0 || value > 32) return PAMG_E_ARG; A->tile_D = value; break;
        case 17: if (value < -1 || value > 4) return PAMG_E_ARG; A->tile_Q = value; break;
        case 18: if (value < 0 || value > 1) return PAMG_E_ARG; A->tile_part = value; break;
        case 19: A->use_idx16 = value != 0; return PAMG_OK;
        case 20: if (value != 0 && (value < 64 || value > 2048)) return PAMG_E_ARG; A->gs_cap = value & ~3; break;
        case 24: if (value < 0 || value > 1) return PAMG_E_ARG; A->gs_order = value; return PAMG_OK;
        case 25: if (value != 0 && value != 4 && value != 8 && value != 16 && value != 32 && value != 64) return PAMG_E_ARG; A->lane_L = value; break;
        case 26: if (value < 0) return PAMG_E_ARG; A->lane_G = value; matrix_drop_point_twin(A); return PAMG_OK;
        case 27: if (value < 0 || value > 1) return PAMG_E_ARG; A->lane_wide = value; matrix_drop_point_twin(A); return PAMG_OK;
        case 33: if (value < 0 || value > 8) return PAMG_E_ARG; A->lane_merge = value; break;
        case 35: if (value < 0 || value > 2) return PAMG_E_ARG; A->lanem_rpw = value; break;
        case 38: if (value != 0 && value != 1 && value != 4 && value != 8) return PAMG_E_ARG; A->lanem_cluster = value; break;
        case 36: if (value < 0 || value > 98304) return PAMG_E_ARG; A->lds_pad = value & ~15; return PAMG_OK;
        case 34: if (value < 1 || value > 400) return PAMG_E_ARG; A->lanem_ahead10 = value; matrix_drop_point_twin(A); return PAMG_OK;
        case 37: if (value < 0 || value > 1) return PAMG_E_ARG; A->sym_fused = value; return PAMG_OK;
        case 30:
            if (value < 0 || value > 2) return PAMG_E_ARG;
            A->line_scan = value;
            matrix_drop_point_twin(A);
            for (int k = 0; k < 4; ++k) if (A->gs[k]) A->gs[k]->line_unfit = false;
            return PAMG_OK;
        case 31: if (value != 2 && value != 4 && value != 8) return PAMG_E_ARG; A->rowmask_kz = value; return PAMG_OK;
        case 32: if (value < 0 || value > 7) return PAMG_E_ARG; A->rowmask_flags = value; return PAMG_OK;
        case 28: if (value < 0 || value > 15 || (value & 6)) return PAMG_E_ARG; A->lane_flags = value; matrix_drop_point_twin(A); return PAMG_OK;
        default: return PAMG_E_ARG;
    }
    if (key == 25 || key == 33 || key == 35 || key == 38) {
        matrix_drop_point_twin(A);
        for (int k = 0; k < 4; ++k) {
            GsSchedule *g = A->gs[k];
            if (g) g->lane_unfit = false;
            if (g && g->lane) { const size_t lb = lane_part_bytes(g); A->bytes -= lb; g->bytes -= lb; free_lane_part(g->lane); g->lane = nullptr; }
            if (g) g->lanem_unfit = false;
            if (g && g->lanem) { const size_t lb = lanem_part_bytes(g); A->bytes -= lb; g->bytes -= lb; free_lanem_part(g->lanem); g->lanem = nullptr; }
            if (g) g->blane_unfit = false;
            if (g && g->blane) { const size_t lb = blane_part_bytes(g); A->bytes -= lb; g->bytes -= lb; free_blane_part(g->blane); g->blane = nullptr; }
            if (g) g->line_unfit = false;
        }
        return PAMG_OK;
    }
    if (key >= 12) {
        for (int k = 0; k < 4; ++k) {
            GsSchedule *g = A->gs[k];
            if (g) g->tile_unfit = false;
            if (g && g->tile) { A->bytes -= g->tile->bytes; g->bytes -= g->tile->bytes; free_tile_part(g->tile); g->tile = nullptr; }
        }
        return PAMG_OK;
    }
    for (int k = 0; k < 4; ++k) { if (A->gs[k]) A->bytes -= A->gs[k]->bytes; free_schedule(A->gs[k]); A->gs[k] = nullptr; }
    matrix_drop_point_twin(A);
    return replan(A);
}

int pamg_matrix_autotune(pamg_matrix_t A, int allow_cap)
{
    if (!A) return PAMG_E_ARG;
    if (A->borrowed > 0) return PAMG_E_STATE;
    if (A->nnz < 4000000 || A->npl != 2) return PAMG_OK;
    const size_t ts = tsize(A->dtype);
    void *x = nullptr, *y = nullptr;
    PAMG_HIP(hipMalloc(&x, (size_t)(A->ncols + 8) * ts));
    if (hipMalloc(&y, (size_t)(A->nrows + 8) * ts) != hipSuccess) { hipFree(x); return (int)hipErrorOutOfMemory; }
    hipMemset(x, 0, (size_t)(A->ncols + 8) * ts);
    hipEvent_t e0, e1;
    hipEventCreate(&e0); hipEventCreate(&e1);
    const int cap0 = A->cap, fl0 = A->stream_flags;
    const int caps[2] = {cap0, 512};
    int best_cap = cap0, best_fl = fl0, st = PAMG_OK;
    float best_ms = 1e30f;
    long long rm0[8];
    const bool masked = pamg_matrix_row_masks(A, rm0) == PAMG_OK && rm0[0] > 0;
    const int idx0 = A->use_idx16;
    const int nidx = (A->d_Aj16 && !A->d_Ax8 && idx0) ? 2 : 1;
    const bool square = A->nrows == A->ncols;
    const int probe = square ? EPI_RESID : EPI_SET;
    void *pb = nullptr;
    if (square) {
        if (hipMalloc(&pb, (size_t)(A->nrows + 8) * ts) != hipSuccess) { hipFree(x); hipFree(y); hipEventDestroy(e0); hipEventDestroy(e1); return (int)hipErrorOutOfMemory; }
        hipMemset(pb, 0, (size_t)(A->nrows + 8) * ts);
    }
    float cand_ms[2][2][2][2];
    for (int q = 0; q < 16; ++q) (&cand_ms[0][0][0][0])[q] = 1e30f;
    const int nvc = A->d_Ax8 ? 1 : 2;
    for (int ci = 0; ci < (allow_cap ? 2 : 1) && st == PAMG_OK && !masked; ++ci) {
        if (caps[ci] != A->cap) { A->cap = caps[ci]; st = replan(A); if (st) break; }
        for (int round = 0; round < 2 && st == PAMG_OK; ++round) {
            for (int ix = 0; ix < nidx && st == PAMG_OK; ++ix) {
                A->use_idx16 = ix == 0 ? idx0 : 0;
                for (int fl = 0; fl < 2 && st == PAMG_OK; ++fl)
                    for (int vc = 0; vc < nvc && st == PAMG_OK; ++vc) {
                        A->stream_flags = (fl0 & ~(1 | 32)) | fl | (vc ? 32 : 0);
                        for (int w = 0; w < 2 && st == PAMG_OK; ++w) st = stream_launch(A, probe, x, pb, y, 0.0, 0.0, nullptr, nullptr);
                        hipEventRecord(e0, nullptr);
                        for (int r = 0; r < 6 && st == PAMG_OK; ++r) st = stream_launch(A, probe, x, pb, y, 0.0, 0.0, nullptr, nullptr);
                        hipEventRecord(e1, nullptr);
                        hipEventSynchronize(e1);
                        float ms = 0.f;
                        hipEventElapsedTime(&ms, e0, e1);
                        if (st == PAMG_OK) cand_ms[ci][ix][fl][vc] = std::min(cand_ms[ci][ix][fl][vc], ms);
                    }
            }
        }
// ... 47 lines not shown
    return st;
}

int pamg_matrix_gs_profile(pamg_matrix_t A, int which, long long *out, int64_t capacity, int64_t *count)
{
    if (!A || which < 0 || which > 3 || !count) return PAMG_E_ARG;
    *count = 0;
    GsSchedule *g = A->gs[which];
    if (g && g->tile && g->tile->d_prof) {
        PAMG_HIP(hipDeviceSynchronize());
        TileSched *t = g->tile;
        *count = t->nsteps;
        if (!out) return PAMG_OK;
        if (capacity < t->nsteps) return PAMG_E_ARG;
        PAMG_HIP(hipMemcpy(out, t->d_prof, (size_t)t->nsteps * 8 * sizeof(long long), hipMemcpyDeviceToHost));
        std::vector<int> ts((size_t)t->G + 1);
        PAMG_HIP(hipMemcpy(ts.data(), t->d_tile_step, ts.size() * sizeof(int), hipMemcpyDeviceToHost));
        for (int k = 0; k < t->G; ++k)
            for (int q = ts[k]; q < ts[k + 1]; ++q) { out[(size_t)q * 8 + 2] = k; out[(size_t)q * 8 + 3] = q - ts[k]; }
        return PAMG_OK;
    }
    if (!g || !g->d_prof) return PAMG_OK;
    PAMG_HIP(hipDeviceSynchronize());
    *count = g->nblk_total;
    if (!out) return PAMG_OK;
    if (capacity < g->nblk_total) return PAMG_E_ARG;
    PAMG_HIP(hipMemcpy(out, g->d_prof, (size_t)g->nblk_total * 8 * sizeof(long long), hipMemcpyDeviceToHost));
    for (int l = 0; l < g->nlevels; ++l)
        for (int q = g->level_blk[l]; q < g->level_blk[l + 1]; ++q) out[(size_t)q * 8 + 7] = l;
    return PAMG_OK;
}

int pamg_matrix_line_info(pamg_matrix_t A, int which, int64_t info[8])
{
    if (!A || which < 0 || which > 3 || !info) return PAMG_E_ARG;
    return pamg::line_info(A->gs[which], info);
}

int pamg_matrix_lane_info(pamg_matrix_t A, int which, int64_t info[8])
{
    if (!A || which < 0 || which > 3 || !info) return PAMG_E_ARG;
    if (A->R > 1) return pamg::blane_info(A->gs[which], info);
    return pamg::lane_info(A->gs[which], info);
}

int pamg_matrix_kz_info(pamg_matrix_t A, int which, int64_t info[8])
{
    if (!A || !info || which < 0 || which > 3) return PAMG_E_ARG;
    return pamg::kz_lane_info(A->ls[which], info);
}

int pamg_matrix_lanem_info(pamg_matrix_t A, int which, int64_t info[20], double *growth)
{
    if (!A || !info || which < 0 || which > 3) return PAMG_E_ARG;
    return pamg::lanem_info(A->gs[which], info, growth);
}

int pamg_matrix_sym_info(pamg_matrix_t A, int64_t info[8])
{
    if (!A || !info) return PAMG_E_ARG;
    for (int k = 0; k < 8; ++k) info[k] = 0;
    info[0] = A->sym_launches; info[1] = A->sym_zero_launches; info[2] = A->sym_form; info[3] = A->sym_grid; info[4] = A->sym_fused;
    info[5] = -1; info[6] = -1;
    if (!A->d_sym_hf[0]) return PAMG_OK;
    PAMG_HIP(hipDeviceSynchronize());
    unsigned w[8] = {0, 0, 0, 0, 0, 0, 0, 0};
    PAMG_HIP(hipMemcpy(w, A->d_sym_sync, sizeof(w), hipMemcpyDeviceToHost));
    std::vector<unsigned long long> h((size_t)A->nrows);
    if (A->nrows) PAMG_HIP(hipMemcpy(h.data(), A->d_sym_hf[w[5] & 1u], (size_t)A->nrows * 8, hipMemcpyDeviceToHost));
    int64_t bad = 0;
    for (unsigned long long v : h) bad += (v != 0x7FF8DEADBEEF5A5Aull);
    info[5] = bad;
    info[6] = 0;
    for (int k = 0; k < 5; ++k) info[6] += w[k] != 0u;
    return PAMG_OK;
}

int pamg_matrix_lanem_levels(pamg_matrix_t A, int which, int64_t *out, int64_t capacity, int64_t *count)
{
    if (!A || !count || which < 0 || which > 3) return PAMG_E_ARG;
    return pamg::lanem_levels(A->gs[which], out, capacity, count);
}

int pamg_matrix_lane_profile(pamg_matrix_t A, int which, long long *out, int64_t capacity, int64_t *count)
{
    if (!A || which < 0 || which > 3 || !count) return PAMG_E_ARG;
    PAMG_HIP(hipDeviceSynchronize());
    if (A->R > 1) return pamg::blane_profile(A->gs[which], out, capacity, count);
    return pamg::lane_profile(A->gs[which], out, capacity, count);
}

int pamg_matrix_tile_info(pamg_matrix_t A, int which, int64_t info[8])
{
    if (!A || which < 0 || which > 3 || !info) return PAMG_E_ARG;
    for (int k = 0; k < 8; ++k) info[k] = 0;
    const GsSchedule *g = A->gs[which];
    if (!g || !g->tile) return PAMG_OK;
    const TileSched *t = g->tile;
    info[0] = t->G; info[1] = t->W; info[2] = (t->NCH + t->NV + 1) | (t->D << 8) | (TILE_VAR[t->wide][2] << 16) | (t->Q << 24); info[3] = t->nsteps;
    info[4] = t->n_local; info[5] = t->n_global; info[6] = t->n_publish; info[7] = t->lds;
    return PAMG_OK;
}

int pamg_matrix_kaczmarz(pamg_matrix_t L, int nr, void *v, const void *b, const void *Dinv, double omega, int sweep,
                         int iterations, void *xout, pamg_stream_t s)
{
    if (!L || iterations < 0 || sweep < PAMG_FORWARD || sweep > PAMG_SYMMETRIC) return PAMG_E_ARG;
    const int n = (int)L->nrows;
    if (n == 0) return PAMG_OK;
    for (int it = 0; it < iterations; ++it) {
        if (sweep != PAMG_BACKWARD) PAMG_TRY(pamg::kaczmarz_sweep(L, nr != 0, v, b, Dinv, omega, 0, n, 1, xout, (hipStream_t)s));
        if (sweep != PAMG_FORWARD) PAMG_TRY(pamg::kaczmarz_sweep(L, nr != 0, v, b, Dinv, omega, n - 1, -1, -1, xout, (hipStream_t)s));
    }
    return PAMG_OK;
}

// ... 112 lines not shown
```

### pyamg_amd/csrc/pamg_solver.hip

```cpp
#include <algorithm>
#include <cmath>
#include <functional>
#include <map>
#include <new>
#include <thread>

#include "pamg_common.h"

using namespace pamg;

namespace {

struct Smoother {
    int kind = PAMG_SMOOTH_NONE;
    int iterations = 1;
    double omega = 1.0;
    int sweep = PAMG_FORWARD;
    std::vector<double> coeffs;
    void *d_Dinv = nullptr;
    int blocksize = 1;
    pamg_matrix_s *AF = nullptr, *AC = nullptr;
    void *wF = nullptr, *wC = nullptr;
    int f_iterations = 1, c_iterations = 1;
    int *iF = nullptr, *iC = nullptr;
// ... 18 lines not shown
int sweep_bounds(const pamg_matrix_s *A, int dir, int &r0, int &r1, int &rs)
{
    const int n = A->R > 1 ? A->n_brow : (int)A->nrows;
    if (dir == PAMG_FORWARD) { r0 = 0; r1 = n; rs = 1; }
    else if (dir == PAMG_BACKWARD) { r0 = n - 1; r1 = -1; rs = -1; }
    else return PAMG_E_ARG;
    return PAMG_OK;
}

bool square_ok(const pamg_matrix_s *A) { return A && A->nrows == A->ncols && A->R == A->C; }

int jacobi_pp(pamg_matrix_s *A, void **px, void **palt, const void *b, double omega, int its, hipStream_t s)
{
    if (!square_ok(A)) return PAMG_E_ARG;
    if (A->nrows == 0) return PAMG_OK;
    for (int it = 0; it < its; ++it) {
        if (A->R > 1)
            PAMG_TRY(block_jacobi_step(A, PNT_JACOBI, nullptr, *px, *palt, b, omega, s));
        else
            PAMG_TRY(stream_launch(A, A->flavour == PAMG_BSR ? EPI_JACOBI_B : EPI_JACOBI, *px, b, *palt,
                                   0.0, omega, nullptr, s));
        std::swap(*px, *palt);
    }
    return PAMG_OK;
}

int block_jacobi_pp(pamg_matrix_s *A, void **px, void **palt, const void *b, const void *Dinv,
                    double omega, int its, hipStream_t s)
{
    if (!square_ok(A) || A->R < 2 || !Dinv) return PAMG_E_ARG;
    for (int it = 0; it < its; ++it) {
        PAMG_TRY(block_jacobi_step(A, BLK_JACOBI, Dinv, *px, *palt, b, omega, s));
        std::swap(*px, *palt);
    }
    return PAMG_OK;
}

int gs_apply(pamg_matrix_s *A, void *x, const void *b, int sweep, double omega, int its, hipStream_t s, bool x_zero = false)
{
    if (!square_ok(A)) return PAMG_E_ARG;
    if (A->nrows == 0) return PAMG_OK;
    auto one = [&](int dir, double om) -> int {
        int r0, r1, rs;
        PAMG_TRY(sweep_bounds(A, dir, r0, r1, rs));
        int epi;
        if (A->R > 1 || A->flavour == PAMG_BSR) epi = EPI_GS_B;
        else epi = (om != 1.0) ? EPI_SOR : EPI_GS;
        return gs_sweep(A, epi, x, b, om, r0, r1, rs, s);
    };
    if (sweep == PAMG_SYMMETRIC) {
        for (int it = 0; it < its; ++it) {
            bool ran = false;
            PAMG_TRY(gs_sweep_symmetric(A, x, b, x_zero && it == 0, s, &ran));
            if (ran) continue;
            PAMG_TRY(one(PAMG_FORWARD, 1.0));
            PAMG_TRY(one(PAMG_BACKWARD, 1.0));
        }
        return PAMG_OK;
    }
    for (int it = 0; it < its; ++it) PAMG_TRY(one(sweep, omega));
    return PAMG_OK;
}

int block_gs_apply(pamg_matrix_s *A, void *x, const void *b, const void *Dinv, int sweep, int its,
                   hipStream_t s)
{
    if (!square_ok(A) || A->R < 2 || !Dinv) return PAMG_E_ARG;
    auto one = [&](int dir) -> int {
        int r0, r1, rs;
        PAMG_TRY(sweep_bounds(A, dir, r0, r1, rs));
        return block_gs_sweep(A, x, b, Dinv, r0, r1, rs, s);
    };
    for (int it = 0; it < its; ++it) {
        if (sweep == PAMG_SYMMETRIC) { PAMG_TRY(one(PAMG_FORWARD)); PAMG_TRY(one(PAMG_BACKWARD)); }
        else PAMG_TRY(one(sweep));
    }
    return PAMG_OK;
}

int poly_apply(pamg_matrix_s *A, void *x, const void *b, void *work, const double *coeffs, int nc,
               int its, int x_is_zero, hipStream_t s)
{
    if (!A || A->nrows != A->ncols || nc < 1 || !coeffs) return PAMG_E_ARG;
    const int64_t n = A->nrows;
    if (n == 0) return PAMG_OK;
    const size_t ts = tsize(A->dtype);
    void *res_buf = work, *h0 = (char *)work + n * ts, *h1 = (char *)work + 2 * n * ts;
    for (int it = 0; it < its; ++it) {
        const void *res = b;
        bool have_h = false;
        if (!(x_is_zero && it == 0)) {
            PAMG_TRY(stream_launch(A, EPI_RESID, x, b, res_buf, nc > 1 ? coeffs[0] : 0.0, 0.0, nc > 1 ? (double *)h0 : nullptr, s));
            res = res_buf;
            have_h = nc > 1;
        }
        if (nc == 1) {
            PAMG_TRY(vec_axpy(A->dtype, n, coeffs[0], res, x, s));
            continue;
        }
        if (!have_h) PAMG_TRY(vec_scale(A->dtype, n, coeffs[0], res, h0, s));
        void *hc = h0, *hn = h1;
        for (int k = 1; k < nc - 1; ++k) {
            PAMG_TRY(stream_launch(A, EPI_AXPBY, hc, res, hn, coeffs[k], 0.0, nullptr, s));
            std::swap(hc, hn);
        }
        PAMG_TRY(stream_launch(A, EPI_ACC_AXPBY, hc, res, x, coeffs[nc - 1], 0.0, nullptr, s));
// ... 69 lines not shown
            }
            return call(sm.sweep == PAMG_FORWARD, sm.iterations);
        }
        case PAMG_SMOOTH_JACOBI_NE:
            for (int it = 0; it < sm.iterations; ++it) {
                PAMG_TRY(stream_launch(sm.Ar ? sm.Ar : L.A, EPI_RESID, L.x, L.b, L.r, 0.0, 0.0, nullptr, s));
                PAMG_TRY(vec_mul(S->dtype, L.n, L.r, sm.d_Dinv, L.r, s));
                PAMG_TRY(stream_launch(sm.At, EPI_ACC, L.r, nullptr, L.x, 0.0, 0.0, nullptr, s));
            }
            return PAMG_OK;
        case PAMG_SMOOTH_CF_JACOBI:
        case PAMG_SMOOTH_FC_JACOBI:
            for (int it = 0; it < sm.iterations; ++it) {
                const bool f_first = sm.kind == PAMG_SMOOTH_FC_JACOBI;
                for (int half = 0; half < 2; ++half) {
                    const bool f = (half == 0) == f_first;
                    pamg_matrix_s *sub = f ? sm.AF : sm.AC;
                    void *w = f ? sm.wF : sm.wC;
                    const int reps = f ? sm.f_iterations : sm.c_iterations;
                    for (int k = 0; k < reps; ++k) PAMG_TRY(jacobi_indexed(sub, L.x, L.b, sm.omega, w, s));
                }
            }
            return PAMG_OK;
        case PAMG_SMOOTH_KRYLOV: return krylov_smooth(S, L, sm, s);
        case PAMG_SMOOTH_SCHWARZ: {
            int nsub = 0;
            { int64_t info[4]; PAMG_TRY(pamg_schwarz_info(sm.sw, info)); nsub = (int)info[0]; }
            for (int it = 0; it < sm.iterations; ++it) {
                if (sm.sweep != PAMG_BACKWARD) PAMG_TRY(schwarz_sweep(sm.sw, L.x, L.b, 0, nsub, 1, s));
                if (sm.sweep != PAMG_FORWARD) PAMG_TRY(schwarz_sweep(sm.sw, L.x, L.b, nsub - 1, -1, -1, s));
            }
            return PAMG_OK;
        }
        case PAMG_SMOOTH_CF_BLOCK_JACOBI:
        case PAMG_SMOOTH_FC_BLOCK_JACOBI:
            for (int it = 0; it < sm.iterations; ++it) {
                const bool f_first = sm.kind == PAMG_SMOOTH_FC_BLOCK_JACOBI;
                for (int half = 0; half < 2; ++half) {
                    const bool f = (half == 0) == f_first;
                    const int reps = f ? sm.f_iterations : sm.c_iterations;
                    for (int k = 0; k < reps; ++k) {
                        PAMG_TRY(block_jacobi_step(L.A, BLK_JACOBI, sm.d_Dinv, L.x, L.xalt, L.b, sm.omega, s));
                        PAMG_TRY(vec_copy_indexed(S->dtype, f ? sm.nF : sm.nC, f ? sm.iF : sm.iC, L.xalt, L.x, s));
                    }
                }
            }
            return PAMG_OK;
    }
    (void)S;
    return PAMG_E_ARG;
}

void drop_graphs(pamg_solver_s *S);
int prebuild_schedules(Level &L, const Smoother &sm);

int check_sweeps(pamg_solver_s *S)
{
    bool any = false;
    for (Level &L : S->levels) {
        if (!L.A) continue;
        bool e = false;
        PAMG_TRY(sweep_error(L.A, &e));
        any = any || e;
        for (Smoother *sm : {&L.pre, &L.post}) {
            for (pamg_matrix_s *M : {sm->At, sm->Ar})
                if (M && M != L.A) {
                    bool e2 = false;
                    PAMG_TRY(sweep_error(M, &e2));
                    any = any || e2;
                }
            if (sm->sw) {
                bool e3 = false;
                PAMG_TRY(schwarz_error(sm->sw, &e3));
                any = any || e3;
            }
        }
    }
    static int forced = [] { const char *e = getenv("PAMG_FORCE_TIMEOUT"); return e ? atoi(e) : 0; }();
    if (forced > 0) { --forced; any = true; }
    return any ? PAMG_E_TIMEOUT : PAMG_OK;
}

int fall_back_to_level_launches(pamg_solver_s *S)
{
    hipDeviceSynchronize();
    drop_graphs(S);
    for (Level &L : S->levels) {
        if (!L.A) continue;
        L.A->gs_mode = 1;
        L.A->tile_default = false;
        PAMG_TRY(sym_reset(L.A));
        for (Smoother *sm : {&L.pre, &L.post}) {
            if (sm->At) sm->At->gs_mode = 1;
            if (sm->Ar) sm->Ar->gs_mode = 1;
            if (sm->sw) schwarz_level_launches(sm->sw);
            PAMG_TRY(prebuild_schedules(L, *sm));
        }
    }
    S->fallbacks++;
    return PAMG_OK;
}

int coarse_solve(pamg_solver_s *S, const void *b, void *x, hipStream_t s)
{
    if (S->coarse_relax) {
        Level &L = S->levels.back();
        if (b != L.b || x != L.x) return PAMG_E_STATE;
        PAMG_HIP(hipMemsetAsync(L.x, 0, (size_t)L.n * tsize(S->dtype), s));
        PAMG_TRY(apply_smoother(S, L, L.pre, true, s));
        if (L.x != L.x_home) {
            PAMG_HIP(hipMemcpyAsync(L.x_home, L.x, (size_t)L.n * tsize(S->dtype), hipMemcpyDeviceToDevice, s));
            std::swap(L.x, L.xalt);
        }
        return PAMG_OK;
    }
    if (S->coarse_zero) return (int)hipMemsetAsync(x, 0, (size_t)S->n_c * tsize(S->dtype), s);
    if (S->coarse_host) {
        const size_t vb = (size_t)S->n_c * tsize(S->dtype);
        PAMG_HIP(hipMemcpyAsync(S->coarse_hb.data(), b, vb, hipMemcpyDeviceToHost, s));
        PAMG_HIP(hipStreamSynchronize(s));
        if (S->coarse_host(S->coarse_host_user, S->coarse_hb.data(), S->coarse_hx.data(), (int64_t)S->n_c) != 0) return PAMG_E_STATE;
        PAMG_HIP(hipMemcpyAsync(x, S->coarse_hx.data(), vb, hipMemcpyHostToDevice, s));
        PAMG_HIP(hipStreamSynchronize(s));
        return PAMG_OK;
    }
    return dense_gemv(S->dtype, S->n_c, S->d_coarse, b, x, s);
}

int cycle_rec(pamg_solver_s *S, int lvl, int type, int cpl, bool x_zero, hipStream_t s)
{
    Level &L = S->levels[lvl];
    Level &N = S->levels[lvl + 1];
    const int nlev = (int)S->levels.size();
    const size_t ts = tsize(S->dtype);
    PAMG_TRY(apply_smoother(S, L, L.pre, x_zero, s));
    PAMG_TRY(stream_launch(L.A, EPI_RESID, L.x, L.b, L.r, 0.0, 0.0, nullptr, s));
    PAMG_TRY(stream_launch(L.R, EPI_SET, L.r, nullptr, N.b, 0.0, 0.0, reinterpret_cast<double *>(N.x), s));
    if (lvl == nlev - 2) {
        PAMG_TRY(coarse_solve(S, N.b, N.x, s));
    } else if (type == PAMG_CYCLE_V) {
        PAMG_TRY(cycle_rec(S, lvl + 1, PAMG_CYCLE_V, 1, true, s));
    } else if (type == PAMG_CYCLE_W) {
        PAMG_TRY(cycle_rec(S, lvl + 1, PAMG_CYCLE_W, cpl, true, s));
        PAMG_TRY(cycle_rec(S, lvl + 1, PAMG_CYCLE_W, cpl, false, s));
// ... 28 lines not shown
        PAMG_HIP(hipMemcpyAsync(N.x, acc, (size_t)nc * ts, hipMemcpyDeviceToDevice, s));
    } else {
        return PAMG_E_ARG;
    }
    PAMG_TRY(stream_launch(L.P, EPI_ACC, N.x, nullptr, L.x, 0.0, 0.0, nullptr, s));
    PAMG_TRY(apply_smoother(S, L, L.post, false, s));
    if (L.x != L.x_home) {
        PAMG_HIP(hipMemcpyAsync(L.x_home, L.x, (size_t)L.n * ts, hipMemcpyDeviceToDevice, s));
        std::swap(L.x, L.xalt);
    }
    return PAMG_OK;
}

int enqueue_cycle(pamg_solver_s *S, int type, int cpl, bool check, bool x_zero, hipStream_t s)
{
    Level &L0 = S->levels[0];
    if (S->levels.size() == 1) {
        PAMG_TRY(coarse_solve(S, L0.b, L0.x, s));
    } else {
        PAMG_TRY(cycle_rec(S, 0, type, cpl, x_zero, s));
    }
    if (!check) return PAMG_OK;
    PAMG_TRY(stream_launch(L0.A, EPI_SUMSQ, L0.x, L0.b, nullptr, 0.0, 0.0, L0.A->d_partial, s));
    return reduce_partials(L0.A->d_partial, L0.A->nblk, S->d_slot, s);
}

int run_cycle(pamg_solver_s *S, int type, int cpl, hipStream_t s, bool check = true, bool x_zero = false)
{
    if (!S->use_graph || S->host_sync) return enqueue_cycle(S, type, cpl, check, x_zero, s);
    const int key = ((type * 1024 + cpl) * 2 + (check ? 1 : 0)) * 2 + (x_zero ? 1 : 0);
    auto it = S->graphs.find(key);
    if (it == S->graphs.end()) {
        hipGraph_t g = nullptr;
        PAMG_HIP(hipStreamBeginCapture(s, hipStreamCaptureModeThreadLocal));
        const int st = enqueue_cycle(S, type, cpl, check, x_zero, s);
        const hipError_t e = hipStreamEndCapture(s, &g);
        if (st != PAMG_OK) { if (g) hipGraphDestroy(g); return st; }
        if (e != hipSuccess) return (int)e;
        hipGraphExec_t ex = nullptr;
        PAMG_HIP(hipGraphInstantiate(&ex, g, nullptr, nullptr, 0));
        hipGraphDestroy(g);
        it = S->graphs.emplace(key, ex).first;
    }
    return (int)hipGraphLaunch(it->second, s);
}

int ensure_amli(pamg_solver_s *S, int cycle);

static bool sor_takes_omega(const pamg_matrix_s *A, const Smoother &sm)
{
    return sm.kind == PAMG_SMOOTH_SOR && A->R == 1 && A->flavour != PAMG_BSR && sm.sweep != PAMG_SYMMETRIC && sm.omega != 1.0;
}

int prebuild_schedules(Level &L, const Smoother &sm)
{
    if (sm.kind == PAMG_SMOOTH_GS_NE || sm.kind == PAMG_SMOOTH_GS_NR) {
        pamg_matrix_s *Lm = sm.kind == PAMG_SMOOTH_GS_NE ? (sm.Ar ? sm.Ar : L.A) : sm.At;
        const int n = (int)Lm->nrows;
        if (n == 0) return PAMG_OK;
        if (sm.sweep != PAMG_BACKWARD) PAMG_TRY(ensure_line_schedule(Lm, 0, n, 1));
        if (sm.sweep != PAMG_FORWARD) PAMG_TRY(ensure_line_schedule(Lm, n - 1, -1, -1));
        return PAMG_OK;
    }
    const bool gs = sm.kind == PAMG_SMOOTH_GS || sm.kind == PAMG_SMOOTH_SOR || sm.kind == PAMG_SMOOTH_BLOCK_GS;
    if (!gs || L.A->nrows == 0) return PAMG_OK;
    if (sor_takes_omega(L.A, sm) && L.A->lane_merge == 0) L.A->lane_merge = 1;
    int r0, r1, rs;
    if (sm.sweep == PAMG_FORWARD || sm.sweep == PAMG_SYMMETRIC) {
        PAMG_TRY(sweep_bounds(L.A, PAMG_FORWARD, r0, r1, rs));
        PAMG_TRY(ensure_schedule(L.A, r0, r1, rs, sm.kind == PAMG_SMOOTH_BLOCK_GS));
    }
    if (sm.sweep == PAMG_BACKWARD || sm.sweep == PAMG_SYMMETRIC) {
        PAMG_TRY(sweep_bounds(L.A, PAMG_BACKWARD, r0, r1, rs));
        PAMG_TRY(ensure_schedule(L.A, r0, r1, rs, sm.kind == PAMG_SMOOTH_BLOCK_GS));
    }
    if (sm.sweep == PAMG_SYMMETRIC && sm.kind != PAMG_SMOOTH_BLOCK_GS) PAMG_TRY(ensure_sym_parts(L.A));
    return PAMG_OK;
}

struct SchedJob { pamg_matrix_s *A; int r0, r1, rs; int st; bool block_gs; };

void sched_jobs_of(Level &L, const Smoother &sm, std::vector<SchedJob> &jobs)
{
    const bool gs = sm.kind == PAMG_SMOOTH_GS || sm.kind == PAMG_SMOOTH_SOR || sm.kind == PAMG_SMOOTH_BLOCK_GS;
    if (!gs || L.A->nrows == 0) return;
    auto add = [&](int dir) {
        int r0, r1, rs;
        if (sweep_bounds(L.A, dir, r0, r1, rs)) return;
        for (const SchedJob &j : jobs) if (j.A == L.A && j.r0 == r0 && j.r1 == r1 && j.rs == rs && j.block_gs == (sm.kind == PAMG_SMOOTH_BLOCK_GS)) return;
        jobs.push_back({L.A, r0, r1, rs, PAMG_OK, sm.kind == PAMG_SMOOTH_BLOCK_GS});
    };
    if (sm.sweep == PAMG_FORWARD || sm.sweep == PAMG_SYMMETRIC) add(PAMG_FORWARD);
    if (sm.sweep == PAMG_BACKWARD || sm.sweep == PAMG_SYMMETRIC) add(PAMG_BACKWARD);
}

int run_sched_jobs(std::vector<SchedJob> &jobs)
{
    if (jobs.empty()) return PAMG_OK;
    int dev = 0;
    PAMG_HIP(hipGetDevice(&dev));
    const char *e = getenv("PAMG_SCHED_THREADS");
    const bool serial = (e && *e == '1' && !e[1]) || jobs.size() == 1;
    if (serial) {
        for (SchedJob &j : jobs) PAMG_TRY(ensure_schedule(j.A, j.r0, j.r1, j.rs, j.block_gs));
        return PAMG_OK;
    }
    std::vector<std::thread> th;
    for (SchedJob &j : jobs)
        th.emplace_back([&j, dev] {
            j.st = (int)hipSetDevice(dev);
            if (!j.st) j.st = ensure_schedule(j.A, j.r0, j.r1, j.rs, j.block_gs);
        });
    for (auto &t : th) t.join();
    for (const SchedJob &j : jobs) if (j.st) return j.st;
    return PAMG_OK;
}

int dalloc(pamg_solver_s *S, void **p, size_t bytes)
{
    PAMG_HIP(hipMalloc(p, std::max<size_t>(bytes, 256)));
    PAMG_HIP(hipMemset(*p, 0, std::max<size_t>(bytes, 256)));
    S->bytes += std::max<size_t>(bytes, 256);
    return PAMG_OK;
}

int ensure_amli(pamg_solver_s *S, int cycle)
{
    if (cycle != PAMG_CYCLE_AMLI) return PAMG_OK;
    for (size_t l = 1; l < S->levels.size(); ++l) {
        Level &L = S->levels[l];
        if (!L.amli) PAMG_TRY(dalloc(S, &L.amli, 4 * (size_t)L.n * tsize(S->dtype)));
    }
    return PAMG_OK;
}

void drop_graphs(pamg_solver_s *S)
{
    for (auto &kv : S->graphs) hipGraphExecDestroy(kv.second);
    S->graphs.clear();
}


int cg_core(pamg_solver_s *S, pamg_matrix_s *Aop, int64_t n, const std::function<int(const void *, void *)> *precond, void *r, void *z,
            void *p, void *q, void *x, const void *b, double tol, int maxiter, double *residuals, int *n_iter, int *info, hipStream_t s)
{
    const int dt = S->dtype;
    const size_t vb = (size_t)n * tsize(dt);
    if (maxiter <= 0) maxiter = (int)(1.3 * (double)n) + 2;
    if (!precond) z = r;
    double *slot = S->d_slot;
    double h[3];
    auto fetch = [&](int k) -> int {
        PAMG_HIP(hipMemcpyAsync(h, slot + 1, sizeof(double) * (size_t)k, hipMemcpyDeviceToHost, s));
        return (int)hipStreamSynchronize(s);
    };
    PAMG_TRY(stream_launch(Aop, EPI_RESID, x, b, r, 0.0, 0.0, nullptr, s));
    if (precond) PAMG_TRY((*precond)(r, z));
    PAMG_HIP(hipMemcpyAsync(p, z, vb, hipMemcpyDeviceToDevice, s));
    PAMG_TRY(vec_dot(dt, n, r, z, S->d_scratch, slot + 1, s));
    PAMG_TRY(vec_sumsq(dt, n, r, S->d_scratch, slot + 2, s));
    PAMG_TRY(vec_sumsq(dt, n, b, S->d_scratch, slot + 3, s));
    PAMG_TRY(fetch(3));
    double rz = h[0], normr = std::sqrt(h[1]), normb = std::sqrt(h[2]);
    if (normb == 0.0) normb = 1.0;
// ... 884 lines not shown

int pamg_solver_set_coarse_host(pamg_solver_t S, pamg_coarse_host_fn fn, void *user, int n_c)
{
    if (!S || !fn || n_c < 1) return PAMG_E_ARG;
    if (S->finalized) return PAMG_E_STATE;
    S->coarse_host = fn; S->coarse_host_user = user;
    S->n_c = n_c; S->coarse_set = true; S->coarse_zero = false; S->coarse_relax = false;
    S->coarse_hb.assign((size_t)n_c * tsize(S->dtype), 0);
    S->coarse_hx.assign((size_t)n_c * tsize(S->dtype), 0);
    S->host_sync = true;
    return PAMG_OK;
}

int pamg_solver_set_coarse_relax(pamg_solver_t S)
{
    if (!S || S->levels.empty()) return PAMG_E_ARG;
    if (S->finalized) return PAMG_E_STATE;
    if (S->levels.back().P) return PAMG_E_STATE;
    if (S->levels.back().pre.kind == PAMG_SMOOTH_NONE) return PAMG_E_ARG;
    S->coarse_relax = true; S->coarse_set = true; S->coarse_zero = false;
    S->coarse_host = nullptr; S->coarse_host_user = nullptr;
    recompute_host_sync(S);
    S->n_c = (int)S->levels.back().n;
    return PAMG_OK;
}

int pamg_solver_finalize(pamg_solver_t S)
{
    if (!S || S->levels.empty()) return PAMG_E_ARG;
    if (S->finalized) return PAMG_OK;
    if (S->levels.back().P) return PAMG_E_STATE;
    if (!S->coarse_set || S->n_c != S->levels.back().n) return PAMG_E_STATE;
    const size_t ts = tsize(S->dtype);
    const int nlev = (int)S->levels.size();
    for (int l = 0; l < nlev; ++l) {
        Level &L = S->levels[l];
        const size_t vb = (size_t)L.n * ts;
        PAMG_TRY(dalloc(S, &L.x, vb));
        PAMG_TRY(dalloc(S, &L.xalt, vb));
        PAMG_TRY(dalloc(S, &L.b, vb));
        L.x_home = L.x;
        if (l < nlev - 1 || S->coarse_relax) {
            PAMG_TRY(dalloc(S, &L.r, vb));
            if (L.pre.kind == PAMG_SMOOTH_POLY || L.post.kind == PAMG_SMOOTH_POLY) PAMG_TRY(dalloc(S, &L.work, 3 * vb));
        }
    }
    const int nsm = S->coarse_relax ? nlev : nlev - 1;
    for (int l = 0; l < nsm; ++l) {
        Level &L = S->levels[l];
        if ((sor_takes_omega(L.A, L.pre) || sor_takes_omega(L.A, L.post)) && L.A->lane_merge == 0) L.A->lane_merge = 1;
    }
    {
        std::vector<SchedJob> jobs;
        for (int l = 0; l < nsm; ++l) { sched_jobs_of(S->levels[l], S->levels[l].pre, jobs); sched_jobs_of(S->levels[l], S->levels[l].post, jobs); }
        PAMG_TRY(run_sched_jobs(jobs));
    }
    for (int l = 0; l < nsm; ++l) {
        Level &L = S->levels[l];
        PAMG_TRY(prebuild_schedules(L, L.pre));
        PAMG_TRY(prebuild_schedules(L, L.post));
    }
    PAMG_TRY(dalloc(S, (void **)&S->d_slot, 16 * sizeof(double)));
    PAMG_TRY(dalloc(S, (void **)&S->d_scratch, 1032 * sizeof(double)));
    PAMG_HIP(hipStreamCreateWithFlags(&S->own_stream, hipStreamNonBlocking));
    S->finalized = true;
    return PAMG_OK;
}

int pamg_solver_set_graph(pamg_solver_t S, int enable)
{
    if (!S) return PAMG_E_ARG;
    S->use_graph = enable != 0;
    if (!S->use_graph) drop_graphs(S);
    return PAMG_OK;
}

int pamg_solver_cycle(pamg_solver_t S, void *x, const void *b, int cycle, int cycles_per_level, pamg_stream_t s_)
{
    if (!S || !x || !b) return PAMG_E_ARG;
    if (!S->finalized) return PAMG_E_STATE;
    if (cycle < PAMG_CYCLE_V || cycle > PAMG_CYCLE_AMLI || cycles_per_level < 1 || cycles_per_level > 1023) return PAMG_E_ARG;
    hipStream_t s = s_ ? (hipStream_t)s_ : S->own_stream;
    PAMG_TRY(ensure_amli(S, cycle));
    if (!s_) PAMG_HIP(hipStreamSynchronize(nullptr));
    Level &L0 = S->levels[0];
    const size_t vb = (size_t)L0.n * tsize(S->dtype);
    PAMG_HIP(hipMemcpyAsync(L0.x, x, vb, hipMemcpyDeviceToDevice, s));
    PAMG_HIP(hipMemcpyAsync(L0.b, b, vb, hipMemcpyDeviceToDevice, s));
    PAMG_TRY(run_cycle(S, cycle, cycles_per_level, s));
    PAMG_HIP(hipMemcpyAsync(x, L0.x, vb, hipMemcpyDeviceToDevice, s));
    if (!s_) PAMG_HIP(hipStreamSynchronize(s));
    return PAMG_OK;
}

}

namespace pamg {
int solver_cycle_inline(pamg_solver_s *S, void *x, const void *b, int cycle, int cpl, hipStream_t s, bool allow_graph)
{
    if (!S || !x || !b || !s) return PAMG_E_ARG;
    if (!S->finalized) return PAMG_E_STATE;
    if (cycle == PAMG_CYCLE_AMLI) return PAMG_E_UNSUPPORTED;
    Level &L0 = S->levels[0];
    const size_t vb = (size_t)L0.n * tsize(S->dtype);
    PAMG_HIP(hipMemcpyAsync(L0.x, x, vb, hipMemcpyDeviceToDevice, s));
    PAMG_HIP(hipMemcpyAsync(L0.b, b, vb, hipMemcpyDeviceToDevice, s));
    if (allow_graph) PAMG_TRY(run_cycle(S, cycle, cpl, s, false, false));
    else PAMG_TRY(enqueue_cycle(S, cycle, cpl, false, false, s));
    PAMG_HIP(hipMemcpyAsync(x, L0.x, vb, hipMemcpyDeviceToDevice, s));
    return PAMG_OK;
}

// ... 239 lines not shown
```

### pyamg_amd/multilevel.py

```python
from __future__ import annotations

import ctypes as C
from typing import List, Optional

import numpy as np

from . import _capi as capi
from .hierarchy import HierarchySpec, SmootherSpec, SparseOp, extract

__all__ = ["DeviceMatrix", "DeviceMultilevelSolver"]


class DeviceMatrix:

    def __init__(self, op: SparseOp):
        lib = capi.lib()
        self.op = op
        self.dtype = np.dtype(op.dtype)
        R, Cc = op.blocksize
        h = C.c_void_p()
        capi.check(lib.pamg_matrix_create(
            C.byref(h), capi.dtype_code(op.dtype), capi.BSR if op.fmt == "bsr" else capi.CSR,
            op.shape[0] // R, op.shape[1] // Cc, R, Cc,
            capi.ptr(op.indptr), capi.ptr(op.indices), capi.ptr(op.data)), "pamg_matrix_create")
# ... 52 lines not shown

    def row_patterns(self) -> int:
        n = C.c_int(0)
        capi.check(capi.lib().pamg_matrix_row_patterns(self.handle, C.byref(n)), "pamg_matrix_row_patterns")
        return int(n.value)

    def row_masks(self) -> dict:
        out = (C.c_longlong * 8)()
        capi.check(capi.lib().pamg_matrix_row_masks(self.handle, out), "pamg_matrix_row_masks")
        keys = ("entries", "walked_rows", "lattice", "line", "plane", "planes_per_lane", "flags", "launch_grid")
        return dict(zip(keys, (int(v) for v in out)))

    def tile_info(self, which=0):
        a = (C.c_int64 * 8)()
        capi.check(capi.lib().pamg_matrix_tile_info(self.handle, which, a), "pamg_matrix_tile_info")
        d = dict(zip(("tiles", "ring", "geom", "steps", "early_local", "early_global", "publishing_rows", "lds_bytes"), list(a)))
        geom = d.pop("geom")
        d.update(code_chunks=geom & 0xFF, lds_slots=(geom >> 8) & 0xFF, gather_depth=(geom >> 16) & 0xFF, loader_in_flight=(geom >> 24) & 0xFF)
        return d

    def lane_info(self, which=0):
        a = (C.c_int64 * 8)()
        capi.check(capi.lib().pamg_matrix_lane_info(self.handle, which, a), "pamg_matrix_lane_info")
        return dict(zip(("lanes_per_row", "slots_per_lane", "groups", "entry_slots", "early_entries", "launch_grid", "widest_level_groups", "bytes"), list(a)))

    def lanem_info(self, which=0):
        a = (C.c_int64 * 20)()
        gr = C.c_double(0.0)
        capi.check(capi.lib().pamg_matrix_lanem_info(self.handle, which, a, C.byref(gr)), "pamg_matrix_lanem_info")
        d = dict(zip(("super_levels", "dependency_levels", "rows", "units", "early_operands", "old_operands", "b_operands", "longest_row", "s_max",
                      "closed_by_length", "closed_by_growth", "launch_grid", "cluster_rows", "groups", "padded_slots", "unique_units",
                      "unique_early", "unique_old", "unique_b", "early_lines"), list(a)))
        d["max_growth"] = gr.value
        d["padding"] = d["padded_slots"] / max(1, d["early_operands"] + d["old_operands"] + d["b_operands"])
        return d

    def point_twin(self) -> int:
        st = C.c_int(0)
        capi.check(capi.lib().pamg_matrix_point_twin(self.handle, C.byref(st)), "pamg_matrix_point_twin")
        return int(st.value)

    def lanem_levels(self, which=0):
        n = C.c_int64(0)
        lib = capi.lib()
        capi.check(lib.pamg_matrix_lanem_levels(self.handle, which, None, 0, C.byref(n)), "pamg_matrix_lanem_levels")
        out = np.zeros(n.value, dtype=np.int64)
        if n.value:
            capi.check(lib.pamg_matrix_lanem_levels(self.handle, which, C.c_void_p(out.ctypes.data), n.value, C.byref(n)), "pamg_matrix_lanem_levels")
        return out

    def sym_info(self):
        a = (C.c_int64 * 8)()
        capi.check(capi.lib().pamg_matrix_sym_info(self.handle, a), "pamg_matrix_sym_info")
        d = dict(zip(("launches", "zero_launches", "form", "launch_grid", "enabled", "handoff_not_sentinel", "counters_not_zero"), list(a)[:7]))
        d["form"] = {0: "none", 1: "merged", 2: "line", 3: "merged_one_xcd"}[d["form"]]
        return d

    def line_info(self, which=0):
        a = (C.c_int64 * 8)()
        capi.check(capi.lib().pamg_matrix_line_info(self.handle, which, a), "pamg_matrix_line_info")
        return dict(zip(("slots_per_row", "chunks", "lines", "line_levels", "early_entries", "launch_grid", "widest_level_lines", "bytes"), list(a)))

    def kz_info(self, which=0):
        a = (C.c_int64 * 8)()
        capi.check(capi.lib().pamg_matrix_kz_info(self.handle, which, a), "pamg_matrix_kz_info")
        return dict(zip(("lanes_per_line", "slots_per_lane", "groups", "dependency_levels", "widest_level_groups", "launch_grid", "bytes"), list(a)[:7]))

    def lane_profile(self, which=0):
        n = C.c_int64(0)
        lib = capi.lib()
        capi.check(lib.pamg_matrix_lane_profile(self.handle, which, None, 0, C.byref(n)), "pamg_matrix_lane_profile")
        out = np.zeros((n.value, 4), dtype=np.int64)
        if n.value:
            capi.check(lib.pamg_matrix_lane_profile(self.handle, which, C.c_void_p(out.ctypes.data), n.value, C.byref(n)), "pamg_matrix_lane_profile")
        return out

    def tune(self, lds_entries=None, nnz_per_lane=None, max_rows=None, flow_cap=None, gs_mode=None, gran_cap=None, gran_xcd=None, stream_flags=None, gs_prof=None,
             tile_G=None, tile_W=None, tile_cap=None, tile_default=None, tile_D=None, tile_Q=None, tile_part=None, idx16=None, gs_cap=None, val8=None, rowgather=None, rowpat=None,
             gs_order=None, lane_L=None, lane_G=None, lane_wide=None, lane_flags=None, line_scan=None, rowmask_kz=None, rowmask_flags=None, lane_merge=None, lanem_ahead=None, lanem_rpw=None, lds_pad=None, sym_fused=None, lanem_cluster=None):
        lib = capi.lib()
        for key, v in ((0, lds_entries), (1, nnz_per_lane), (2, max_rows), (3, flow_cap), (5, gs_mode), (6, gran_cap), (7, gran_xcd), (8, stream_flags), (11, gs_prof),
                       (12, tile_G), (13, tile_W), (14, tile_cap), (15, tile_default), (16, tile_D), (17, tile_Q), (18, tile_part), (19, idx16), (20, gs_cap), (21, val8), (22, rowgather), (23, rowpat),
                       (24, gs_order), (25, lane_L), (26, lane_G), (27, lane_wide), (28, lane_flags), (30, line_scan), (31, rowmask_kz), (32, rowmask_flags), (33, lane_merge), (34, lanem_ahead), (35, lanem_rpw), (36, lds_pad), (37, sym_fused), (38, lanem_cluster)):
            if v is not None:
                capi.check(lib.pamg_matrix_tune(self.handle, key, int(v)), "pamg_matrix_tune")

    def spmv(self, mode, x, y, b=None, c=0.0, stream=None, part=None):
        if part is not None:
            capi.check(capi.lib().pamg_matrix_spmv_part(self.handle, int(part), mode, x.ptr, b.ptr if b is not None else None,
                                                        float(c), y.ptr, stream), "pamg_matrix_spmv_part")
            return
        capi.check(capi.lib().pamg_matrix_spmv(self.handle, mode, x.ptr, b.ptr if b is not None else None,
                                               float(c), y.ptr, stream), "pamg_matrix_spmv")

    def split_ranges(self, n_owned_cols: int):
        capi.check(capi.lib().pamg_matrix_split_ranges(self.handle, int(n_owned_cols)), "pamg_matrix_split_ranges")

    def resid_sumsq(self, x, b, out, stream=None):
        capi.check(capi.lib().pamg_matrix_resid_sumsq(self.handle, x.ptr, b.ptr, out.ptr, stream),
                   "pamg_matrix_resid_sumsq")

    def jacobi(self, x, b, work, omega, iterations=1, stream=None):
        capi.check(capi.lib().pamg_matrix_jacobi(self.handle, x.ptr, b.ptr, work.ptr, float(omega),
                                                 int(iterations), stream), "pamg_matrix_jacobi")

    def gauss_seidel(self, x, b, sweep="forward", omega=1.0, iterations=1, stream=None):
        capi.check(capi.lib().pamg_matrix_gauss_seidel(self.handle, x.ptr, b.ptr, capi.SWEEP[sweep],
                                                       float(omega), int(iterations), stream),
                   "pamg_matrix_gauss_seidel")

    def gauss_seidel_x0(self, x, b, sweep="symmetric", omega=1.0, iterations=1, x_is_zero=False, stream=None):
        capi.check(capi.lib().pamg_matrix_gauss_seidel_x0(self.handle, x.ptr, b.ptr, capi.SWEEP[sweep], float(omega), int(iterations),
                                                          int(bool(x_is_zero)), stream), "pamg_matrix_gauss_seidel_x0")

    def polynomial(self, x, b, work, coefficients, iterations=1, x_is_zero=False, stream=None):
        co = np.ascontiguousarray(coefficients, dtype=np.float64)
        capi.check(capi.lib().pamg_matrix_polynomial(self.handle, x.ptr, b.ptr, work.ptr, capi.ptr(co),
                                                     co.size, int(iterations), int(bool(x_is_zero)), stream),
                   "pamg_matrix_polynomial")

    def block_jacobi(self, x, b, work, Dinv, omega, iterations=1, stream=None):
        capi.check(capi.lib().pamg_matrix_block_jacobi(self.handle, x.ptr, b.ptr, work.ptr, Dinv.ptr,
                                                       float(omega), int(iterations), stream),
                   "pamg_matrix_block_jacobi")

    def block_gauss_seidel(self, x, b, Dinv, sweep="forward", iterations=1, stream=None):
        capi.check(capi.lib().pamg_matrix_block_gauss_seidel(self.handle, x.ptr, b.ptr, Dinv.ptr,
                                                             capi.SWEEP[sweep], int(iterations), stream),
                   "pamg_matrix_block_gauss_seidel")

    def free(self):
        if getattr(self, "handle", None):
            try:
                capi._lib.pamg_matrix_destroy(self.handle)
            except Exception:
                pass
# ... 506 lines not shown
```

Measured before the change: 85.15 cycles/s.

## Add zero-initial-guess symmetric GS path using triangular-split merged plans

Adds a specialised symmetric Gauss-Seidel sweep for the first pre-smoothing iteration when x starts at zero. It builds separate lower and upper triangular merged-lane plans and stores the forward-sweep numerator (b minus the lower sum) in a side buffer, so the backward sweep can reuse it instead of recomputing the full row product. This is meant to cut the gathers and arithmetic in the zero-start sweep. In exchange it uses extra plan memory and a new workspace vector and takes longer to set up. By default it is off on the finest level and only used on coarser levels.

```diff
diff --git a/pyamg_amd/csrc/pamg_common.h b/pyamg_amd/csrc/pamg_common.h
--- a/pyamg_amd/csrc/pamg_common.h
+++ b/pyamg_amd/csrc/pamg_common.h
@@ -225,8 +225,17 @@
     unsigned *d_sym_sync = nullptr;
     int sym_cap = 0;
     const void *sym_cap_kernel = nullptr;
+    int zsym_cap = 0;
+    const void *zsym_cap_kernel = nullptr;
+    int sym_general_grid = 0;
     int sym_form = 0, sym_grid = 0;
     long long sym_launches = 0, sym_zero_launches = 0;
+    int zero_plans = 0;
+    int zero_merge = 0;
+    struct pamg::LaneMSched *zplan[2] = {nullptr, nullptr};
+    void *d_zw = nullptr;
+    size_t zero_bytes = 0;
+    long long zero_plan_launches = 0;
     size_t bytes = 0;
 };
 
@@ -338,6 +347,15 @@
 int lanem_info(const GsSchedule *g, int64_t *info, double *growth);
 int lanem_levels(const GsSchedule *g, int64_t *out, int64_t cap, int64_t *n);
 int lanem_sym_launch(pamg_matrix_s *A, GsSchedule *gf, GsSchedule *gb, void *x, const void *b, bool x_zero, hipStream_t s);
+int lanem_plan_info(const struct LaneMSched *t, int64_t *info, double *growth);
+int build_zero_plan(pamg_matrix_s *A, int dir);
+void free_zero_plans(pamg_matrix_s *A);
+size_t zero_plan_bytes(const pamg_matrix_s *A);
+bool zero_plans_ready(const pamg_matrix_s *A, const GsSchedule *gf, const GsSchedule *gb);
+int lanem_zero_pair_launch(pamg_matrix_s *A, GsSchedule *gf, GsSchedule *gb, void *x, const void *b, hipStream_t s);
+int ensure_zero_parts(pamg_matrix_s *A, bool build);
+void matrix_drop_zero_plans(pamg_matrix_s *A);
+int gs_sweep_zero_pair(pamg_matrix_s *A, void *x, const void *b, hipStream_t s, bool *ran);
 int sym_fill_sentinels(void *p, int64_t n);
 int sweep_error(pamg_matrix_s *A, bool *error);
 inline size_t tsize(int dtype) { return dtype == PAMG_F64 ? 8 : 4; }
diff --git a/pyamg_amd/csrc/pamg_lane.hip b/pyamg_amd/csrc/pamg_lane.hip
--- a/pyamg_amd/csrc/pamg_lane.hip
+++ b/pyamg_amd/csrc/pamg_lane.hip
@@ -1,6 +1,7 @@
 #include "pamg_common.h"
 #include "pamg_lane_plan.h"
 #include "pamg_lanem_plan.h"
+#include "pamg_tile_plan.h"
 
 namespace pamg {
 
@@ -343,6 +344,7 @@
     const int *crid;
     const double *crd;
     int crows;
+    double *w;
 };
 
 __global__ __launch_bounds__(BLK) void lanem_prepare_kernel(const double *__restrict__ x, double *__restrict__ xold, double *__restrict__ xs, int64_t n)
@@ -359,6 +361,7 @@
     int c[NREG];
     double v[NREG], xv[NREG];
     double bv, xo, rd;
+    double num;
     int rid;
     int gate, unit, K, g;
 };
@@ -393,7 +396,7 @@
     }
 }
 
-template <int NREG>
+template <int NREG, bool BCOH = false>
 __device__ __forceinline__ void m_gather(const LaneMArgs &a, MCtx<NREG> &C, int idle, const bool xz = false, const bool coh = false)
 {
 #pragma unroll
@@ -405,7 +408,8 @@
             if (!(C.c[k] & (LANE_EARLY | LANEM_BSRC))) C.c[k] |= LANE_NONE;
     }
     const int row = C.rid < 0 ? 0 : (C.rid & LANE_MASK);
-    C.bv = a.b[row];
+    if constexpr (BCOH) C.bv = __hip_atomic_load(a.b + row, __ATOMIC_RELAXED, __HIP_MEMORY_SCOPE_AGENT);
+    else C.bv = a.b[row];
     C.xo = coh ? __hip_atomic_load(a.xold + row, __ATOMIC_RELAXED, __HIP_MEMORY_SCOPE_AGENT) : a.xold[row];
 #pragma unroll
     for (int k = 0; k < NREG; ++k) {
@@ -486,12 +490,13 @@
     }
     s = seg_allreduce<64 / RPW, T>(s);
     const bool upd = C.rid >= 0 && !(C.rid & LANE_NODIAG);
-    T val = (C.bv - s) * C.rd;
+    C.num = C.bv - s;
+    T val = C.num * C.rd;
     if (!upd) val = C.xo;
     return val;
 }
 
-template <int RPW, int MODE, int NREG, int PH = 0>
+template <int RPW, int MODE, int NREG, int PH = 0, bool WST = false>
 __device__ __forceinline__ void m_publish(const LaneMArgs &a, const MCtx<NREG> &C, double val)
 {
     if (((threadIdx.x & 63) & (64 / RPW - 1)) == 0 && C.rid >= 0) {
@@ -501,6 +506,9 @@
         if constexpr (PH != 1) {
             if (!(C.rid & LANE_NODIAG)) a.y[row] = val;
         }
+        if constexpr (WST) {
+            if (!(C.rid & LANE_NODIAG)) __hip_atomic_store(a.w + row, C.num, __ATOMIC_RELAXED, __HIP_MEMORY_SCOPE_AGENT);
+        }
     }
 }
 
@@ -508,7 +516,7 @@
 
 __device__ __forceinline__ int4 c_rec(const int4 *rp, int g, int gend) { return rp[(size_t)(g < gend ? g : gend - 1)]; }
 
-template <int PH>
+template <int PH, bool WST = false, bool BCOH = false>
 __device__ __forceinline__ void c_group(const LaneMArgs &a, double *lds, const int4 &q, int g, int lane, int idle, const bool xz, const bool coh)
 {
     using T = double;
@@ -549,7 +557,9 @@
     const int rid = unused ? -1 : a.crid[ri];
     const T rd = a.crd[ri];
     const int row = rid < 0 ? 0 : (rid & LANE_MASK);
-    const T bv = a.b[row];
+    T bv;
+    if constexpr (BCOH) bv = __hip_atomic_load(a.b + row, __ATOMIC_RELAXED, __HIP_MEMORY_SCOPE_AGENT);
+    else bv = a.b[row];
     const T xo = coh ? __hip_atomic_load(a.xold + row, __ATOMIC_RELAXED, __HIP_MEMORY_SCOPE_AGENT) : a.xold[row];
     unsigned pend = 0;
 #pragma unroll
@@ -611,17 +621,21 @@
     __builtin_amdgcn_fence(__ATOMIC_RELEASE, "wavefront");
     __builtin_amdgcn_wave_barrier();
     const bool upd = rid >= 0 && !(rid & LANE_NODIAG);
-    T val = (bv - s) * rd;
+    const T num = bv - s;
+    T val = num * rd;
     if (!upd) val = xo;
     if (tail && rid >= 0) {
         __hip_atomic_store(a.xs + row, val, __ATOMIC_RELAXED, __HIP_MEMORY_SCOPE_AGENT);
         if constexpr (PH != 1) {
             if (upd) a.y[row] = val;
         }
-    }
-}
-
-template <int MODE, int RPW, int NREG>
+        if constexpr (WST) {
+            if (upd) __hip_atomic_store(a.w + row, num, __ATOMIC_RELAXED, __HIP_MEMORY_SCOPE_AGENT);
+        }
+    }
+}
+
+template <int MODE, int RPW, int NREG, int Z = 0>
 __global__ __launch_bounds__(BLK) void gs_lanem_kernel(const LaneMArgs a)
 {
     const int lane = threadIdx.x & 63;
@@ -638,7 +652,7 @@
         int4 q = c_rec(rp, g, gend);
         for (; g < gend; g += W) {
             const int4 nq = c_rec(rp, g + W, gend);
-            c_group<0>(a, c_lds + wib * LANEC_UMAX, q, g, lane, idle, false, false);
+            c_group<0, Z != 0>(a, c_lds + wib * LANEC_UMAX, q, g, lane, idle, false, false);
             q = nq;
         }
     } else {
@@ -661,7 +675,7 @@
                 long long t2 = 0;
                 unsigned sp = 0;
                 const double val = m_finish<RPW, NREG>(a, X, idle, &t2, &sp);
-                m_publish<RPW, MODE, NREG>(a, X, val);
+                m_publish<RPW, MODE, NREG, 0, Z != 0>(a, X, val);
                 if (lane == 0) {
                     long long *o = a.prof + (size_t)g * 4;
                     o[0] = t0 | ((long long)(sp > 4095u ? 4095u : sp) << 52);
@@ -671,7 +685,7 @@
                 m_slots<RPW, NREG>(a, X, q0, q1, g, lane);
                 m_gather<NREG>(a, X, idle);
                 const double val = m_finish<RPW, NREG>(a, X, idle);
-                m_publish<RPW, MODE, NREG>(a, X, val);
+                m_publish<RPW, MODE, NREG, 0, Z != 0>(a, X, val);
             }
             q0 = n0; q1 = n1;
         }
@@ -701,7 +715,7 @@
             m_slots<RPW, NREG>(a, X, q0, q1, g, lane);
             m_gather<NREG>(a, X, idle);
             const double val = m_finish<RPW, NREG>(a, X, idle);
-            m_publish<RPW, MODE, NREG>(a, X, val);
+            m_publish<RPW, MODE, NREG, 0, Z != 0>(a, X, val);
             if (g2 >= gend) break;
             g = g2; q0 = n0; q1 = n1;
             g2 = (int)__builtin_amdgcn_readfirstlane(tk3);
@@ -731,7 +745,7 @@
     }
 }
 
-template <int MODE, int RPW, int NREG, int PH>
+template <int MODE, int RPW, int NREG, int PH, int Z = 0>
 __device__ __forceinline__ unsigned m_phase(const LaneMArgs &a, double *wipe, int wq, int wr, int wblk, unsigned *ticket, const bool xz, int lane, int wib, int idle, double *c_lds)
 {
     const int4 *rp = reinterpret_cast<const int4 *>(a.rec);
@@ -745,7 +759,7 @@
         int4 q = c_rec(rp, g, gend);
         for (; g < gend; g += W) {
             const int4 nq = c_rec(rp, g + W, gend);
-            c_group<PH>(a, c_lds + wib * LANEC_UMAX, q, g, lane, idle, xz, PH == 2);
+            c_group<PH, Z && PH == 1, Z && PH == 2>(a, c_lds + wib * LANEC_UMAX, q, g, lane, idle, xz, PH == 2);
             m_wipe<MODE>(wipe, g, gend, wq, wr, wblk, lane);
             ++done;
             q = nq;
@@ -762,9 +776,9 @@
             int4 n0, n1;
             m_rec(rp, g + W, gend, n0, n1);
             m_slots<RPW, NREG>(a, X, q0, q1, g, lane);
-            m_gather<NREG>(a, X, idle, xz, PH == 2);
+            m_gather<NREG, Z && PH == 2>(a, X, idle, xz, PH == 2);
             const double val = m_finish<RPW, NREG>(a, X, idle, nullptr, nullptr, xz);
-            m_publish<RPW, MODE, NREG, PH>(a, X, val);
+            m_publish<RPW, MODE, NREG, PH, Z && PH == 1>(a, X, val);
             m_wipe<MODE>(wipe, g, gend, wq, wr, wblk, lane);
             ++done;
             q0 = n0; q1 = n1;
@@ -784,9 +798,9 @@
             unsigned tk3 = 0;
             if (g2 < gend && lane == 0) tk3 = __hip_atomic_fetch_add(ticket, 1u, __ATOMIC_RELAXED, __HIP_MEMORY_SCOPE_AGENT);
             m_slots<RPW, NREG>(a, X, q0, q1, g, lane);
-            m_gather<NREG>(a, X, idle, xz, PH == 2);
+            m_gather<NREG, Z && PH == 2>(a, X, idle, xz, PH == 2);
             const double val = m_finish<RPW, NREG>(a, X, idle, nullptr, nullptr, xz);
-            m_publish<RPW, MODE, NREG, PH>(a, X, val);
+            m_publish<RPW, MODE, NREG, PH, Z && PH == 1>(a, X, val);
             m_wipe<MODE>(wipe, g, gend, wq, wr, wblk, lane);
             ++done;
             if (g2 >= gend) break;
@@ -830,7 +844,7 @@
     }
 }
 
-template <int MODE, int RPW, int NREG>
+template <int MODE, int RPW, int NREG, int Z = 0>
 __global__ __launch_bounds__(BLK) void gs_lanem_sym_kernel(const LaneMSymArgs a)
 {
     __shared__ unsigned sh_done;
@@ -856,9 +870,9 @@
         LaneMArgs p1 = a.ph[0], p2 = a.ph[1];
         p1.xs = hf; p1.y = nullptr;
         p2.xold = hf;
-        const unsigned done = m_phase<MODE, RPW, NREG, 1>(p1, p2.xs, a.wq[0], a.wr[0], a.wblk[0], a.sync + 2, a.xzero != 0, lane, wib, idle, c_lds);
+        const unsigned done = m_phase<MODE, RPW, NREG, 1, Z>(p1, p2.xs, a.wq[0], a.wr[0], a.wblk[0], a.sync + 2, a.xzero != 0, lane, wib, idle, c_lds);
         sym_phase_barrier(a.sync, p1.err, &sh_done, done, (unsigned)p1.ngroups);
-        (void)m_phase<MODE, RPW, NREG, 2>(p2, hf_next, a.wq[1], a.wr[1], a.wblk[1], a.sync + 3, false, lane, wib, idle, c_lds);
+        (void)m_phase<MODE, RPW, NREG, 2, Z>(p2, hf_next, a.wq[1], a.wr[1], a.wblk[1], a.sync + 3, false, lane, wib, idle, c_lds);
     }
     sym_leave(a.sync, parity);
 }
@@ -1075,6 +1089,8 @@
     return A->nrows > 131072 ? (lanem_cluster_rows(A) ? 4 : 3) : 8;
 }
 
+static int lanem_to_device(const LaneMPlan &P, int s_max, LaneMSched **out);
+
 int build_lanem_part(pamg_matrix_s *A, GsSchedule *g)
 {
     if (g->lanem) return PAMG_OK;
@@ -1091,6 +1107,22 @@
                          s_max, 1e3, P, LANEM_KMAX * 64, rpw, cluster))
         return PAMG_E_ARG;
     hAx = PlanVec<double>();
+    LaneMSched *t = nullptr;
+    PAMG_TRY(lanem_to_device(P, s_max, &t));
+    if (!g->d_xold) {
+        const size_t xb = ((size_t)A->nrows + 8) * sizeof(double);
+        const int st = (int)hipMalloc(&g->d_xold, xb);
+        if (st) { free_lanem_part(t); return st; }
+        t->bytes += xb;
+    }
+    g->lanem = t;
+    g->bytes += t->bytes;
+    return PAMG_OK;
+}
+
+static int lanem_to_device(const LaneMPlan &P, int s_max, LaneMSched **out)
+{
+    *out = nullptr;
     if (P.nsuper * 10 > P.nlevels * 9) return PAMG_E_ARG;
     LaneMSched *t = new (std::nothrow) LaneMSched();
     if (!t) return PAMG_E_ALLOC;
@@ -1112,15 +1144,9 @@
         if (!st) st = lane_upload(&t->d_sidx, P.sidx.data(), P.sidx.size() * sizeof(unsigned short), &t->bytes);
         if (!st) st = lane_upload(&t->d_crid, P.rid.data(), P.rid.size() * sizeof(int), &t->bytes);
         if (!st) st = lane_upload(&t->d_crd, P.rdiag.data(), P.rdiag.size() * sizeof(double), &t->bytes);
-        if (!st && !g->d_xold) {
-            const size_t xb = ((size_t)A->nrows + 8) * sizeof(double);
-            st = (int)hipMalloc(&g->d_xold, xb);
-            if (!st) t->bytes += xb;
-        }
         if (st) { free_lanem_part(t); return st; }
         if (getenv("PAMG_TIMING")) fprintf(stderr, "[pamg timing]     lanem plan: cluster layout, %d rows per wave: %zu bytes uploaded\n", P.cluster, t->bytes);
-        g->lanem = t;
-        g->bytes += t->bytes;
+        *out = t;
         return PAMG_OK;
     }
     std::vector<LaneMRec> rec((size_t)P.ngroups);
@@ -1139,16 +1165,85 @@
     int st = lane_upload(&t->d_rec, rec.data(), rec.size() * sizeof(LaneMRec), &t->bytes);
     if (!st) st = lane_upload(&t->d_cols, P.cols.data(), P.cols.size() * sizeof(int), &t->bytes);
     if (!st) st = lane_upload(&t->d_vals, P.vals.data(), P.vals.size() * sizeof(double), &t->bytes);
-    if (!st && !g->d_xold) {
-        const size_t xb = ((size_t)A->nrows + 8) * sizeof(double);
-        st = (int)hipMalloc(&g->d_xold, xb);
-        if (!st) t->bytes += xb;
-    }
     if (st) { free_lanem_part(t); return st; }
     if (getenv("PAMG_TIMING")) fprintf(stderr, "[pamg timing]     lanem plan: %d row(s) per wave: %zu bytes uploaded\n", P.rpw, t->bytes);
-    g->lanem = t;
-    g->bytes += t->bytes;
+    *out = t;
     return PAMG_OK;
+}
+
+int lanem_zero_smax(const pamg_matrix_s *A)
+{
+    if (A->zero_merge >= 2) return A->zero_merge;
+    static const int env = [] { const char *e = getenv("PAMG_ZERO_MERGE"); return e ? atoi(e) : 0; }();
+    if (env >= 2) return env;
+    return A->nrows > 131072 ? 6 : 16;
+}
+
+int build_zero_plan(pamg_matrix_s *A, int dir)
+{
+    if (dir < 0 || dir > 1 || A->zplan[dir]) return PAMG_OK;
+    if (A->dtype != PAMG_F64 || A->R != 1 || A->nrows < 2 || A->nrows != A->ncols || !A->d_Ax) return PAMG_E_ARG;
+    PhaseTimer pt_(dir ? "build_zero_plan (backward, triu)" : "build_zero_plan (forward, tril)", A->nnz);
+    const int n = (int)A->nrows;
+    PlanVec<double> hAx;
+    hAx.resize((size_t)A->nnz + 1);
+    if (A->nnz) PAMG_HIP(hipMemcpy(hAx.data(), A->d_Ax, (size_t)A->nnz * sizeof(double), hipMemcpyDeviceToHost));
+    const int *Ap = A->h_Ap.data(), *Aj = A->h_Aj.data();
+    std::vector<int> Tp((size_t)n + 1, 0);
+    lane_parallel(n, [&](int64_t i0, int64_t i1) {
+        for (int64_t i = i0; i < i1; ++i) {
+            int c = 0;
+            for (int p = Ap[i]; p < Ap[i + 1]; ++p) c += dir ? (Aj[p] >= (int)i) : (Aj[p] <= (int)i);
+            Tp[(size_t)i + 1] = c;
+        }
+    });
+    for (int i = 0; i < n; ++i) Tp[(size_t)i + 1] += Tp[(size_t)i];
+    PlanVec<int> Tj;
+    PlanVec<double> Tx;
+    Tj.resize((size_t)Tp[(size_t)n] + 1);
+    Tx.resize((size_t)Tp[(size_t)n] + 1);
+    lane_parallel(n, [&](int64_t i0, int64_t i1) {
+        for (int64_t i = i0; i < i1; ++i) {
+            int q = Tp[(size_t)i];
+            for (int p = Ap[i]; p < Ap[i + 1]; ++p)
+                if (dir ? (Aj[p] >= (int)i) : (Aj[p] <= (int)i)) { Tj[(size_t)q] = Aj[p]; Tx[(size_t)q] = hAx[(size_t)p]; ++q; }
+        }
+    });
+    hAx = PlanVec<double>();
+    std::vector<int> vis, lvl;
+    int m = 0, nl = 0;
+    if (sweep_levels(n, Tp.data(), Tj.data(), dir ? n - 1 : 0, dir ? -1 : n, dir ? -1 : 1, vis, lvl, m, nl) || m != n || nl < 8) return PAMG_E_ARG;
+    const int s_max = lanem_zero_smax(A);
+    const int rpw = A->lanem_rpw ? A->lanem_rpw : (A->nrows > 131072 ? 2 : 1);
+    LaneMPlan P;
+    if (build_lanem_plan(n, Tp.data(), Tj.data(), Tx.data(), dir ? n - 1 : 0, dir ? -1 : 1, m, nl, vis, lvl, s_max, 1e3, P, LANEM_KMAX * 64, rpw, lanem_cluster_rows(A)))
+        return PAMG_E_ARG;
+    LaneMSched *t = nullptr;
+    PAMG_TRY(lanem_to_device(P, s_max, &t));
+    A->zplan[dir] = t;
+    return PAMG_OK;
+}
+
+void free_zero_plans(pamg_matrix_s *A)
+{
+    for (int d = 0; d < 2; ++d) { free_lanem_part(A->zplan[d]); A->zplan[d] = nullptr; }
+    hipFree(A->d_zw);
+    A->d_zw = nullptr;
+}
+
+size_t zero_plan_bytes(const pamg_matrix_s *A)
+{
+    size_t b = A->d_zw ? ((size_t)A->nrows + 8) * sizeof(double) : 0;
+    for (int d = 0; d < 2; ++d) if (A->zplan[d]) b += A->zplan[d]->bytes;
+    return b;
+}
+
+bool zero_plans_ready(const pamg_matrix_s *A, const GsSchedule *gf, const GsSchedule *gb)
+{
+    const LaneMSched *zf = A->zplan[0], *zb = A->zplan[1];
+    if (A->zero_plans == 1 || !zf || !zb || !A->d_zw || !gf || !gb || !gf->lanem || !gb->lanem) return false;
+    return zf->rpw == zb->rpw && zf->cluster == zb->cluster && zf->rpw == gf->lanem->rpw && zf->cluster == gf->lanem->cluster &&
+           zb->rpw == gb->lanem->rpw && zb->cluster == gb->lanem->cluster && zf->ngroups >= 1 && zb->ngroups >= 1;
 }
 
 static void lanem_layout_args(const LaneMSched *t, LaneMArgs &a)
@@ -1158,15 +1253,15 @@
     a.sidx = t->d_sidx; a.crid = t->d_crid; a.crd = t->d_crd; a.crows = t->cluster;
 }
 
-int lanem_launch(pamg_matrix_s *A, GsSchedule *g, void *x, const void *b, hipStream_t s)
-{
-    LaneMSched *t = g->lanem;
+static int lanem_launch_plan(pamg_matrix_s *A, GsSchedule *g, LaneMSched *t, void *x, const void *b, double *w, hipStream_t s)
+{
     if (!t || !g->d_xold) return PAMG_E_STATE;
     const int64_t n = A->nrows;
     LaneMArgs a;
     lanem_layout_args(t, a);
     a.use_gate = (A->lane_flags & 1) ? 1 : 0;
     a.xold = (const double *)g->d_xold; a.y = (double *)x; a.xs = (double *)g->d_xs; a.b = (const double *)b;
+    a.w = w;
     a.err = g->d_sync + 1; a.ticket = g->d_sync + 20;
     a.ngroups = (int)t->ngroups;
     a.nidle = (int)std::max<int64_t>(1, std::min<int64_t>(n, 1 << 20));
@@ -1185,6 +1280,11 @@
                   : t->rpw == 2 ? (xcd ? (const void *)gs_lanem_kernel<1, 2, 4> : (const void *)gs_lanem_kernel<0, 2, 4>)
                   : all_regs    ? (xcd ? (const void *)gs_lanem_kernel<1, 1, 8> : (const void *)gs_lanem_kernel<0, 1, 8>)
                                 : (xcd ? (const void *)gs_lanem_kernel<1, 1, 2> : (const void *)gs_lanem_kernel<0, 1, 2>);
+    if (w)
+        k = t->cluster  ? (const void *)gs_lanem_kernel<0, 0, 8, 1>
+          : t->rpw == 2 ? (xcd ? (const void *)gs_lanem_kernel<1, 2, 4, 1> : (const void *)gs_lanem_kernel<0, 2, 4, 1>)
+          : all_regs    ? (xcd ? (const void *)gs_lanem_kernel<1, 1, 8, 1> : (const void *)gs_lanem_kernel<0, 1, 8, 1>)
+                        : (xcd ? (const void *)gs_lanem_kernel<1, 1, 2, 1> : (const void *)gs_lanem_kernel<0, 1, 2, 1>);
     static thread_local int cus = 0;
     if (!cus) cus = device_cus_lane();
     if (!(t->cap > 0 && t->cap_kernel == k)) {
@@ -1213,6 +1313,17 @@
     return PAMG_OK;
 }
 
+int lanem_launch(pamg_matrix_s *A, GsSchedule *g, void *x, const void *b, hipStream_t s) { return lanem_launch_plan(A, g, g->lanem, x, b, nullptr, s); }
+
+int lanem_zero_pair_launch(pamg_matrix_s *A, GsSchedule *gf, GsSchedule *gb, void *x, const void *b, hipStream_t s)
+{
+    if (!zero_plans_ready(A, gf, gb)) return PAMG_E_UNSUPPORTED;
+    PAMG_TRY(lanem_launch_plan(A, gf, A->zplan[0], x, b, (double *)A->d_zw, s));
+    PAMG_TRY(lanem_launch_plan(A, gb, A->zplan[1], x, A->d_zw, nullptr, s));
+    A->zero_plan_launches++;
+    return PAMG_OK;
+}
+
 int sym_fill_sentinels(void *p, int64_t n)
 {
     if (n <= 0) return PAMG_OK;
@@ -1227,18 +1338,21 @@
 {
     LaneMSched *tf = gf->lanem, *tb = gb->lanem;
     if (!tf || !tb || !A->d_sym_hf[0] || !A->d_sym_hf[1] || !A->d_sym_hb || !A->d_sym_sync) return PAMG_E_STATE;
+    const bool zero = x_zero && zero_plans_ready(A, gf, gb);
+    if (zero) { tf = A->zplan[0]; tb = A->zplan[1]; }
     const int64_t n = A->nrows;
     auto one_xcd = [&](const GsSchedule *g) { return !g->lanem->cluster && (A->gran_xcd == 1 || (A->gran_xcd == 0 && lane_one_xcd(A, g) && A->nrows <= 8192)); };
     const bool xcd = one_xcd(gf);
     if (xcd != one_xcd(gb) || tf->rpw != tb->rpw || tf->cluster != tb->cluster || tf->ngroups < 1 || tb->ngroups < 1) return PAMG_E_UNSUPPORTED;
     LaneMSymArgs a;
-    GsSchedule *gs2[2] = {gf, gb};
+    LaneMSched *ts2[2] = {tf, tb};
     for (int p = 0; p < 2; ++p) {
-        LaneMSched *t = gs2[p]->lanem;
+        LaneMSched *t = ts2[p];
         LaneMArgs &q = a.ph[p];
         lanem_layout_args(t, q);
         q.use_gate = (A->lane_flags & 1) ? 1 : 0;
         q.b = (const double *)b;
+        q.w = nullptr;
         q.err = gf->d_sync + 1; q.ticket = nullptr;
         q.ngroups = (int)t->ngroups;
         q.nidle = (int)std::max<int64_t>(1, std::min<int64_t>(n, 1 << 20));
@@ -1249,6 +1363,7 @@
     }
     a.ph[0].xold = (const double *)x; a.ph[0].y = nullptr;     a.ph[0].xs = nullptr;
     a.ph[1].xold = nullptr;           a.ph[1].y = (double *)x; a.ph[1].xs = (double *)A->d_sym_hb;
+    if (zero) { a.ph[0].w = (double *)A->d_zw; a.ph[1].b = (const double *)A->d_zw; }
     a.hf[0] = (double *)A->d_sym_hf[0]; a.hf[1] = (double *)A->d_sym_hf[1];
     a.sync = A->d_sym_sync;
     a.xzero = x_zero ? 1 : 0;
@@ -1258,18 +1373,25 @@
                   : tf->rpw == 2 ? (xcd ? (const void *)gs_lanem_sym_kernel<1, 2, 4> : (const void *)gs_lanem_sym_kernel<0, 2, 4>)
                   : all_regs     ? (xcd ? (const void *)gs_lanem_sym_kernel<1, 1, 8> : (const void *)gs_lanem_sym_kernel<0, 1, 8>)
                                  : (xcd ? (const void *)gs_lanem_sym_kernel<1, 1, 2> : (const void *)gs_lanem_sym_kernel<0, 1, 2>);
+    if (zero)
+        k = tf->cluster  ? (const void *)gs_lanem_sym_kernel<0, 0, 8, 1>
+          : tf->rpw == 2 ? (xcd ? (const void *)gs_lanem_sym_kernel<1, 2, 4, 1> : (const void *)gs_lanem_sym_kernel<0, 2, 4, 1>)
+          : all_regs     ? (xcd ? (const void *)gs_lanem_sym_kernel<1, 1, 8, 1> : (const void *)gs_lanem_sym_kernel<0, 1, 8, 1>)
+                         : (xcd ? (const void *)gs_lanem_sym_kernel<1, 1, 2, 1> : (const void *)gs_lanem_sym_kernel<0, 1, 2, 1>);
     static thread_local int cus = 0;
     if (!cus) cus = device_cus_lane();
-    if (!(A->sym_cap > 0 && A->sym_cap_kernel == k)) {
+    int &kcap = zero ? A->zsym_cap : A->sym_cap;
+    const void *&kcap_kernel = zero ? A->zsym_cap_kernel : A->sym_cap_kernel;
+    if (!(kcap > 0 && kcap_kernel == k)) {
         int nb = 0;
         if (hipOccupancyMaxActiveBlocksPerMultiprocessor(&nb, k, BLK, 0) != hipSuccess) nb = 2;
-        A->sym_cap = std::max(1, std::min(nb - 1, 8));
-        A->sym_cap_kernel = k;
-    }
-    const int cap = A->sym_cap;
+        kcap = std::max(1, std::min(nb - 1, 8));
+        kcap_kernel = k;
+    }
+    const int cap = kcap;
     int G = 1;
     for (int p = 0; p < 2; ++p) {
-        const LaneMSched *t = gs2[p]->lanem;
+        const LaneMSched *t = ts2[p];
         const int per_level = (int)((t->ngroups + t->nsuper - 1) / std::max(1, t->nsuper));
         const int64_t want_waves = std::max<int64_t>(128, ((int64_t)A->lanem_ahead10 * per_level + 9) / 10);
         int Gp = (int)std::min<int64_t>((want_waves + LANE_WPB - 1) / LANE_WPB, (int64_t)std::min(cap, (t->rpw == 2 || t->cluster) ? 2 : 3) * cus);
@@ -1281,17 +1403,21 @@
     void *args[] = {(void *)&a};
     PAMG_HIP(hipLaunchKernel(k, dim3(G), dim3(BLK), args, 0, s));
     A->sym_form = xcd ? 3 : 1; A->sym_grid = G;
+    if (zero) tf->last_grid = tb->last_grid = G;
+    else A->sym_general_grid = G;
     A->sym_launches++;
     if (x_zero) A->sym_zero_launches++;
+    if (zero) A->zero_plan_launches++;
     return PAMG_OK;
 }
 
-int lanem_info(const GsSchedule *g, int64_t *info, double *growth)
+int lanem_info(const GsSchedule *g, int64_t *info, double *growth) { return lanem_plan_info(g ? g->lanem : nullptr, info, growth); }
+
+int lanem_plan_info(const LaneMSched *t, int64_t *info, double *growth)
 {
     for (int i = 0; i < 20; ++i) info[i] = 0;
     if (growth) *growth = 0.0;
-    if (!g || !g->lanem) return PAMG_OK;
-    const LaneMSched *t = g->lanem;
+    if (!t) return PAMG_OK;
     info[0] = t->nsuper; info[1] = t->nlevels; info[2] = t->nrows; info[3] = t->n_units; info[4] = t->n_early; info[5] = t->n_old; info[6] = t->n_b;
     info[7] = t->max_len; info[8] = t->s_max; info[9] = t->closed_by_length; info[10] = t->closed_by_growth; info[11] = t->last_grid;
     info[12] = t->cluster; info[13] = t->ngroups; info[14] = t->n_units * 64; info[15] = t->n_uunits;
diff --git a/pyamg_amd/csrc/pamg_matrix.hip b/pyamg_amd/csrc/pamg_matrix.hip
--- a/pyamg_amd/csrc/pamg_matrix.hip
+++ b/pyamg_amd/csrc/pamg_matrix.hip
@@ -821,6 +821,7 @@
         free_schedule(g);
         if (l) free_line_schedule(l);
     }
+    matrix_drop_zero_plans(A);
     matrix_drop_point_twin(A);
 }
 
@@ -1323,7 +1324,87 @@
         PAMG_TRY(ensure_sym_parts(A));
         if (!A->d_sym_hf[0]) return PAMG_OK;
     }
+    if (form == 1 && x_zero && A->zero_plans == 2 && !A->zplan[0] && !A->zplan[1]) {
+        hipStreamCaptureStatus cs = hipStreamCaptureStatusNone;
+        PAMG_HIP(hipStreamIsCapturing(s, &cs));
+        if (cs == hipStreamCaptureStatusNone) {
+            PAMG_TRY(ensure_zero_parts(A, true));
+            if (!zero_plans_ready(A, gf, gb)) A->zero_plans = 1;
+        }
+    }
     const int st = form == 2 ? line_sym_launch(A, gf, gb, x, b, s) : lanem_sym_launch(A, gf, gb, x, b, x_zero, s);
+    if (st == PAMG_E_UNSUPPORTED) return PAMG_OK;
+    if (st == PAMG_OK) *ran = true;
+    return st;
+}
+
+void matrix_drop_zero_plans(pamg_matrix_s *A)
+{
+    if (!A || (!A->zplan[0] && !A->zplan[1] && !A->d_zw)) return;
+    free_zero_plans(A);
+    std::lock_guard<std::mutex> lk(g_sched_mu);
+    A->bytes -= std::min(A->bytes, A->zero_bytes);
+    A->zero_bytes = 0;
+}
+
+static bool zero_form_of(pamg_matrix_s *A, GsSchedule **pf, GsSchedule **pb)
+{
+    if (A->zero_plans == 1 || A->R != 1 || A->dtype != PAMG_F64 || A->gs_order != 1 || A->gs_mode != 0 || A->gs_prof || A->nrows < 2) return false;
+    const int n = (int)A->nrows;
+    GsSchedule *gf = nullptr, *gb = nullptr;
+    if (get_schedule(A, 0, n, 1, &gf) != PAMG_OK || get_schedule(A, n - 1, -1, -1, &gb) != PAMG_OK) return false;
+    if (ensure_parts(A, gf) != PAMG_OK || ensure_parts(A, gb) != PAMG_OK) return false;
+    if (gf->nrows != A->nrows || gb->nrows != A->nrows) return false;
+    if (want_lines(A, gf) || want_lines(A, gb)) return false;
+    if (!(want_lanes(A, gf) && want_lanes(A, gb) && gf->lanem && gb->lanem)) return false;
+    *pf = gf; *pb = gb;
+    return true;
+}
+
+int ensure_zero_parts(pamg_matrix_s *A, bool build)
+{
+    if (!A) return PAMG_OK;
+    GsSchedule *gf = nullptr, *gb = nullptr;
+    if (!zero_form_of(A, &gf, &gb)) { matrix_drop_zero_plans(A); return PAMG_OK; }
+    if (A->d_zw && A->zplan[0] && A->zplan[1]) return PAMG_OK;
+    if (build && (!A->zplan[0] || !A->zplan[1])) {
+        int st[2] = {PAMG_OK, PAMG_OK};
+        int dev = 0;
+        PAMG_HIP(hipGetDevice(&dev));
+        std::thread other([&] { st[1] = (int)hipSetDevice(dev); if (!st[1]) st[1] = build_zero_plan(A, 1); });
+        st[0] = build_zero_plan(A, 0);
+        other.join();
+        for (int d = 0; d < 2; ++d) if (st[d] != PAMG_OK && st[d] != PAMG_E_ARG) { matrix_drop_zero_plans(A); return st[d]; }
+    }
+    if (!A->zplan[0] || !A->zplan[1]) { matrix_drop_zero_plans(A); return PAMG_OK; }
+    if (!A->d_zw) {
+        const size_t vb = ((size_t)A->nrows + 8) * sizeof(double);
+        PAMG_HIP(hipMalloc(&A->d_zw, vb));
+        PAMG_HIP(hipMemset(A->d_zw, 0, vb));
+    }
+    if (!zero_plans_ready(A, gf, gb)) { matrix_drop_zero_plans(A); return PAMG_OK; }
+    std::lock_guard<std::mutex> lk(g_sched_mu);
+    A->bytes -= std::min(A->bytes, A->zero_bytes);
+    A->zero_bytes = zero_plan_bytes(A);
+    A->bytes += A->zero_bytes;
+    return PAMG_OK;
+}
+
+int gs_sweep_zero_pair(pamg_matrix_s *A, void *x, const void *b, hipStream_t s, bool *ran)
+{
+    *ran = false;
+    if (A->zero_plans == 1 || (A->zero_plans == 0 && !A->zplan[0])) return PAMG_OK;
+    GsSchedule *gf = nullptr, *gb = nullptr;
+    if (!zero_form_of(A, &gf, &gb)) return PAMG_OK;
+    if (!zero_plans_ready(A, gf, gb)) {
+        if (A->zero_plans != 2 || A->zplan[0] || A->zplan[1]) return PAMG_OK;
+        hipStreamCaptureStatus cs = hipStreamCaptureStatusNone;
+        PAMG_HIP(hipStreamIsCapturing(s, &cs));
+        if (cs != hipStreamCaptureStatusNone) return PAMG_OK;
+        PAMG_TRY(ensure_zero_parts(A, true));
+        if (!zero_plans_ready(A, gf, gb)) { A->zero_plans = 1; return PAMG_OK; }
+    }
+    const int st = lanem_zero_pair_launch(A, gf, gb, x, b, s);
     if (st == PAMG_E_UNSUPPORTED) return PAMG_OK;
     if (st == PAMG_OK) *ran = true;
     return st;
@@ -1796,6 +1877,7 @@
     for (int k = 0; k < 4; ++k) free_schedule(A->gs[k]);
     for (int k = 0; k < 4; ++k) pamg::free_line_schedule(A->ls[k]);
     hipFree(A->d_sym_hf[0]); hipFree(A->d_sym_hf[1]); hipFree(A->d_sym_hb); hipFree(A->d_sym_sync);
+    pamg::free_zero_plans(A);
     if (A->point_twin) pamg_matrix_destroy(A->point_twin);
     delete A;
     return PAMG_OK;
@@ -1891,6 +1973,8 @@
         case 36: if (value < 0 || value > 98304) return PAMG_E_ARG; A->lds_pad = value & ~15; return PAMG_OK;
         case 34: if (value < 1 || value > 400) return PAMG_E_ARG; A->lanem_ahead10 = value; matrix_drop_point_twin(A); return PAMG_OK;
         case 37: if (value < 0 || value > 1) return PAMG_E_ARG; A->sym_fused = value; return PAMG_OK;
+        case 39: if (value < 0 || value > 2) return PAMG_E_ARG; A->zero_plans = value; if (value == 1) matrix_drop_zero_plans(A); return PAMG_OK;
+        case 40: if (value != 0 && (value < 2 || value > 16)) return PAMG_E_ARG; A->zero_merge = value; matrix_drop_zero_plans(A); return PAMG_OK;
         case 30:
             if (value < 0 || value > 2) return PAMG_E_ARG;
             A->line_scan = value;
@@ -1904,6 +1988,7 @@
     }
     if (key == 25 || key == 33 || key == 35 || key == 38) {
         matrix_drop_point_twin(A);
+        matrix_drop_zero_plans(A);
         for (int k = 0; k < 4; ++k) {
             GsSchedule *g = A->gs[k];
             if (g) g->lane_unfit = false;
@@ -1925,6 +2010,7 @@
         return PAMG_OK;
     }
     for (int k = 0; k < 4; ++k) { if (A->gs[k]) A->bytes -= A->gs[k]->bytes; free_schedule(A->gs[k]); A->gs[k] = nullptr; }
+    matrix_drop_zero_plans(A);
     matrix_drop_point_twin(A);
     return replan(A);
 }
@@ -2078,7 +2164,8 @@
 
 int pamg_matrix_lanem_info(pamg_matrix_t A, int which, int64_t info[20], double *growth)
 {
-    if (!A || !info || which < 0 || which > 3) return PAMG_E_ARG;
+    if (!A || !info || which < 0 || which > 5) return PAMG_E_ARG;
+    if (which >= 4) return pamg::lanem_plan_info(A->zplan[which - 4], info, growth);
     return pamg::lanem_info(A->gs[which], info, growth);
 }
 
@@ -2086,8 +2173,9 @@
 {
     if (!A || !info) return PAMG_E_ARG;
     for (int k = 0; k < 8; ++k) info[k] = 0;
-    info[0] = A->sym_launches; info[1] = A->sym_zero_launches; info[2] = A->sym_form; info[3] = A->sym_grid; info[4] = A->sym_fused;
+    info[0] = A->sym_launches; info[1] = A->sym_zero_launches; info[2] = A->sym_form; info[3] = A->sym_general_grid ? A->sym_general_grid : A->sym_grid; info[4] = A->sym_fused;
     info[5] = -1; info[6] = -1;
+    info[7] = A->zero_plan_launches;
     if (!A->d_sym_hf[0]) return PAMG_OK;
     PAMG_HIP(hipDeviceSynchronize());
     unsigned w[8] = {0, 0, 0, 0, 0, 0, 0, 0};
diff --git a/pyamg_amd/csrc/pamg_solver.hip b/pyamg_amd/csrc/pamg_solver.hip
--- a/pyamg_amd/csrc/pamg_solver.hip
+++ b/pyamg_amd/csrc/pamg_solver.hip
@@ -94,6 +94,8 @@
         for (int it = 0; it < its; ++it) {
             bool ran = false;
             PAMG_TRY(gs_sweep_symmetric(A, x, b, x_zero && it == 0, s, &ran));
+            if (ran) continue;
+            if (x_zero && it == 0) PAMG_TRY(gs_sweep_zero_pair(A, x, b, s, &ran));
             if (ran) continue;
             PAMG_TRY(one(PAMG_FORWARD, 1.0));
             PAMG_TRY(one(PAMG_BACKWARD, 1.0));
@@ -269,7 +271,7 @@
 }
 
 void drop_graphs(pamg_solver_s *S);
-int prebuild_schedules(Level &L, const Smoother &sm);
+int prebuild_schedules(Level &L, const Smoother &sm, bool zero = false);
 
 int check_sweeps(pamg_solver_s *S)
 {
@@ -307,6 +309,7 @@
         L.A->gs_mode = 1;
         L.A->tile_default = false;
         PAMG_TRY(sym_reset(L.A));
+        matrix_drop_zero_plans(L.A);
         for (Smoother *sm : {&L.pre, &L.post}) {
             if (sm->At) sm->At->gs_mode = 1;
             if (sm->Ar) sm->Ar->gs_mode = 1;
@@ -441,7 +444,15 @@
     return sm.kind == PAMG_SMOOTH_SOR && A->R == 1 && A->flavour != PAMG_BSR && sm.sweep != PAMG_SYMMETRIC && sm.omega != 1.0;
 }
 
-int prebuild_schedules(Level &L, const Smoother &sm)
+static bool zero_plans_wanted(const pamg_matrix_s *A, const Smoother &pre, const Smoother &post, int l)
+{
+    if (A->zero_plans == 1 || (l == 0 && A->zero_plans != 2)) return false;
+    if (pre.kind != PAMG_SMOOTH_GS || pre.sweep != PAMG_SYMMETRIC || pre.iterations < 1) return false;
+    if (sor_takes_omega(A, post)) return false;
+    return A->R == 1 && A->dtype == PAMG_F64 && A->gs_order == 1 && A->gs_mode == 0 && A->nrows >= 2;
+}
+
+int prebuild_schedules(Level &L, const Smoother &sm, bool zero)
 {
     if (sm.kind == PAMG_SMOOTH_GS_NE || sm.kind == PAMG_SMOOTH_GS_NR) {
         pamg_matrix_s *Lm = sm.kind == PAMG_SMOOTH_GS_NE ? (sm.Ar ? sm.Ar : L.A) : sm.At;
@@ -464,12 +475,24 @@
         PAMG_TRY(ensure_schedule(L.A, r0, r1, rs, sm.kind == PAMG_SMOOTH_BLOCK_GS));
     }
     if (sm.sweep == PAMG_SYMMETRIC && sm.kind != PAMG_SMOOTH_BLOCK_GS) PAMG_TRY(ensure_sym_parts(L.A));
-    return PAMG_OK;
-}
-
-struct SchedJob { pamg_matrix_s *A; int r0, r1, rs; int st; bool block_gs; };
-
-void sched_jobs_of(Level &L, const Smoother &sm, std::vector<SchedJob> &jobs)
+    if (zero) PAMG_TRY(ensure_zero_parts(L.A, true));
+    return PAMG_OK;
+}
+
+struct SchedJob { pamg_matrix_s *A; int r0, r1, rs; int st; bool block_gs; int zero_dir; };
+
+static int sched_job_run(SchedJob &j)
+{
+    PAMG_TRY(ensure_schedule(j.A, j.r0, j.r1, j.rs, j.block_gs));
+    if (j.zero_dir < 0) return PAMG_OK;
+    GsSchedule *g = nullptr;
+    PAMG_TRY(get_schedule(j.A, j.r0, j.r1, j.rs, &g));
+    if (!g || !g->lanem) return PAMG_OK;
+    const int st = build_zero_plan(j.A, j.zero_dir);
+    return st == PAMG_E_ARG ? PAMG_OK : st;
+}
+
+void sched_jobs_of(Level &L, const Smoother &sm, std::vector<SchedJob> &jobs, bool zero = false)
 {
     const bool gs = sm.kind == PAMG_SMOOTH_GS || sm.kind == PAMG_SMOOTH_SOR || sm.kind == PAMG_SMOOTH_BLOCK_GS;
     if (!gs || L.A->nrows == 0) return;
@@ -477,7 +500,7 @@
         int r0, r1, rs;
         if (sweep_bounds(L.A, dir, r0, r1, rs)) return;
         for (const SchedJob &j : jobs) if (j.A == L.A && j.r0 == r0 && j.r1 == r1 && j.rs == rs && j.block_gs == (sm.kind == PAMG_SMOOTH_BLOCK_GS)) return;
-        jobs.push_back({L.A, r0, r1, rs, PAMG_OK, sm.kind == PAMG_SMOOTH_BLOCK_GS});
+        jobs.push_back({L.A, r0, r1, rs, PAMG_OK, sm.kind == PAMG_SMOOTH_BLOCK_GS, zero ? (dir == PAMG_BACKWARD ? 1 : 0) : -1});
     };
     if (sm.sweep == PAMG_FORWARD || sm.sweep == PAMG_SYMMETRIC) add(PAMG_FORWARD);
     if (sm.sweep == PAMG_BACKWARD || sm.sweep == PAMG_SYMMETRIC) add(PAMG_BACKWARD);
@@ -491,14 +514,14 @@
     const char *e = getenv("PAMG_SCHED_THREADS");
     const bool serial = (e && *e == '1' && !e[1]) || jobs.size() == 1;
     if (serial) {
-        for (SchedJob &j : jobs) PAMG_TRY(ensure_schedule(j.A, j.r0, j.r1, j.rs, j.block_gs));
+        for (SchedJob &j : jobs) PAMG_TRY(sched_job_run(j));
         return PAMG_OK;
     }
     std::vector<std::thread> th;
     for (SchedJob &j : jobs)
         th.emplace_back([&j, dev] {
             j.st = (int)hipSetDevice(dev);
-            if (!j.st) j.st = ensure_schedule(j.A, j.r0, j.r1, j.rs, j.block_gs);
+            if (!j.st) j.st = sched_job_run(j);
         });
     for (auto &t : th) t.join();
     for (const SchedJob &j : jobs) if (j.st) return j.st;
@@ -1489,12 +1512,16 @@
     }
     {
         std::vector<SchedJob> jobs;
-        for (int l = 0; l < nsm; ++l) { sched_jobs_of(S->levels[l], S->levels[l].pre, jobs); sched_jobs_of(S->levels[l], S->levels[l].post, jobs); }
+        for (int l = 0; l < nsm; ++l) {
+            Level &L = S->levels[l];
+            sched_jobs_of(L, L.pre, jobs, zero_plans_wanted(L.A, L.pre, L.post, l));
+            sched_jobs_of(L, L.post, jobs);
+        }
         PAMG_TRY(run_sched_jobs(jobs));
     }
     for (int l = 0; l < nsm; ++l) {
         Level &L = S->levels[l];
-        PAMG_TRY(prebuild_schedules(L, L.pre));
+        PAMG_TRY(prebuild_schedules(L, L.pre, zero_plans_wanted(L.A, L.pre, L.post, l)));
         PAMG_TRY(prebuild_schedules(L, L.post));
     }
     PAMG_TRY(dalloc(S, (void **)&S->d_slot, 16 * sizeof(double)));
diff --git a/pyamg_amd/multilevel.py b/pyamg_amd/multilevel.py
--- a/pyamg_amd/multilevel.py
+++ b/pyamg_amd/multilevel.py
@@ -128,7 +128,7 @@
     def sym_info(self):
         a = (C.c_int64 * 8)()
         capi.check(capi.lib().pamg_matrix_sym_info(self.handle, a), "pamg_matrix_sym_info")
-        d = dict(zip(("launches", "zero_launches", "form", "launch_grid", "enabled", "handoff_not_sentinel", "counters_not_zero"), list(a)[:7]))
+        d = dict(zip(("launches", "zero_launches", "form", "launch_grid", "enabled", "handoff_not_sentinel", "counters_not_zero", "zero_plan_launches"), list(a)))
         d["form"] = {0: "none", 1: "merged", 2: "line", 3: "merged_one_xcd"}[d["form"]]
         return d
 
@@ -153,11 +153,11 @@
 
     def tune(self, lds_entries=None, nnz_per_lane=None, max_rows=None, flow_cap=None, gs_mode=None, gran_cap=None, gran_xcd=None, stream_flags=None, gs_prof=None,
              tile_G=None, tile_W=None, tile_cap=None, tile_default=None, tile_D=None, tile_Q=None, tile_part=None, idx16=None, gs_cap=None, val8=None, rowgather=None, rowpat=None,
-             gs_order=None, lane_L=None, lane_G=None, lane_wide=None, lane_flags=None, line_scan=None, rowmask_kz=None, rowmask_flags=None, lane_merge=None, lanem_ahead=None, lanem_rpw=None, lds_pad=None, sym_fused=None, lanem_cluster=None):
+             gs_order=None, lane_L=None, lane_G=None, lane_wide=None, lane_flags=None, line_scan=None, rowmask_kz=None, rowmask_flags=None, lane_merge=None, lanem_ahead=None, lanem_rpw=None, lds_pad=None, sym_fused=None, lanem_cluster=None, zero_plans=None, zero_merge=None):
         lib = capi.lib()
         for key, v in ((0, lds_entries), (1, nnz_per_lane), (2, max_rows), (3, flow_cap), (5, gs_mode), (6, gran_cap), (7, gran_xcd), (8, stream_flags), (11, gs_prof),
                        (12, tile_G), (13, tile_W), (14, tile_cap), (15, tile_default), (16, tile_D), (17, tile_Q), (18, tile_part), (19, idx16), (20, gs_cap), (21, val8), (22, rowgather), (23, rowpat),
-                       (24, gs_order), (25, lane_L), (26, lane_G), (27, lane_wide), (28, lane_flags), (30, line_scan), (31, rowmask_kz), (32, rowmask_flags), (33, lane_merge), (34, lanem_ahead), (35, lanem_rpw), (36, lds_pad), (37, sym_fused), (38, lanem_cluster)):
+                       (24, gs_order), (25, lane_L), (26, lane_G), (27, lane_wide), (28, lane_flags), (30, line_scan), (31, rowmask_kz), (32, rowmask_flags), (33, lane_merge), (34, lanem_ahead), (35, lanem_rpw), (36, lds_pad), (37, sym_fused), (38, lanem_cluster), (39, zero_plans), (40, zero_merge)):
             if v is not None:
                 capi.check(lib.pamg_matrix_tune(self.handle, key, int(v)), "pamg_matrix_tune")
 
```

Result: faster. 91.09 cycles/s, median of 6 (+7.0%).
